# Isabella98Liu/DG-Mesh

Measured on AMD Instinct MI355X. Metric: train-step iters/sec (800x800, ~100k Gaussians), higher is better.
Workload: dtype f32 (f16x3p split products, fp32 accumulate); 1 GPU; D-NeRF jumpingjacks-like cfg2: 800x800, P=100000 Gaussians, deformation MLP on (deform + deform_back, is_blender), 1 frame per rank per step, fixed P (no densification inside the timed region); output heads of both networks scaled x0.01 so that the deformation field is small as after convergence (default init triples every splat's extent); P=100000, W=800, H=800, num_rendered=2808497, visible=95520, mlp_impl=hip, parallelism=dp1 (frame-parallel, flat-bucket all-reduce 27.8 MB)

## Files before the change

dg-mesh_amd/_lib.py:

```python
import ctypes
import os
import subprocess

_HERE = os.path.dirname(os.path.abspath(__file__))
LIB_PATH = os.environ.get("DGM_LIB_PATH") or os.path.join(_HERE, "lib", "libdgmesh_hip.so")
CSRC = os.path.join(_HERE, "csrc")

_c = ctypes
_vp = _c.c_void_p
ALLOC_FN = _c.CFUNCTYPE(_c.c_void_p, _c.c_void_p, _c.c_size_t)


class StateLayout(_c.Structure):
    _fields_ = [(n, _c.c_size_t) for n in (
        "rec", "depth", "radii", "tiles_touched", "offs", "cov3D", "clamped", "block_sums", "hist",
        "tile_count", "tile_offset", "big_list", "counters", "geometry_bytes",
        "inst", "point_list", "slab", "live", "ckpt", "ckpt64", "ulist_full", "binning_bytes",
        "final_T", "n_contrib", "ranges", "nproc", "cfin", "ulist_last", "image_bytes")] + [
        (n, _c.c_int) for n in ("tiles_x", "tiles_y", "n_chunks", "chunk_size")]


class MlpParams(_c.Structure):
    _fields_ = [(n, _c.c_int) for n in ("n_layers", "width", "emb_dim", "t_dim", "skip_layer", "n_out")] + [
        ("W", _vp * 8), ("b", _vp * 8), ("Wh", _vp), ("bh", _vp)]


_f, _i = _c.c_float, _c.c_int
SYMBOLS = {
    "dgm_abi_version": (_i, []),
    "dgm_last_error": (_c.c_char_p, []),
    "dgm_rasterize_forward": (_i, [ALLOC_FN, _vp, ALLOC_FN, _vp, ALLOC_FN, _vp, _i, _i, _i, _vp, _i, _i, _vp, _vp, _vp,
                                   _vp, _vp, _f, _vp, _vp, _vp, _vp, _vp, _f, _f, _i, _vp, _vp, _i, _vp,
                                   _c.POINTER(_i)]),
    "dgm_rasterize_backward": (_i, [_i, _i, _i, _i, _vp, _i, _i, _vp, _vp, _vp, _vp, _f, _vp, _vp, _vp, _vp, _vp, _f, _f,
                                    _vp, _vp, _vp, _vp, _vp, _vp, _vp, _vp, _vp, _vp, _vp, _vp, _vp, _vp, _i, _vp]),
    "dgm_rasterize_forward_split_sh": (_i, [ALLOC_FN, _vp, ALLOC_FN, _vp, ALLOC_FN, _vp, _i, _i, _i, _vp, _i, _i, _vp, _vp, _vp,
                                            _vp, _vp, _vp, _f, _vp, _vp, _vp, _vp, _vp, _f, _f, _i, _vp, _vp, _i, _vp,
                                            _c.POINTER(_i)]),
    "dgm_rasterize_forward_capacity": (_i, [ALLOC_FN, _vp, ALLOC_FN, _vp, ALLOC_FN, _vp, _i, _i, _i, _vp, _i, _i, _vp, _vp, _vp,
                                            _vp, _vp, _vp, _f, _vp, _vp, _vp, _vp, _vp, _f, _f, _i, _vp, _vp, _i, _vp,
                                            _i, _vp]),
    "dgm_rasterize_backward_split_sh": (_i, [_i, _i, _i, _i, _vp, _i, _i, _vp, _vp, _vp, _vp, _vp, _f, _vp, _vp, _vp, _vp,
                                             _vp, _f, _f, _vp, _vp, _vp, _vp, _vp, _vp, _vp, _vp, _vp, _vp, _vp, _vp, _vp,
                                             _vp, _vp, _i, _vp]),
    "dgm_mark_visible": (_i, [_i, _vp, _vp, _vp, _vp, _vp]),
    "dgm_geometry_bytes": (_c.c_size_t, [_i, _i, _i]),
    "dgm_binning_bytes": (_c.c_size_t, [_i]),
    "dgm_image_bytes": (_c.c_size_t, [_i, _i]),
    "dgm_describe_state": (_i, [_i, _i, _i, _i, _c.POINTER(StateLayout)]),
    "dgm_set_profiling": (None, [_i]),
    "dgm_set_profiling_sampling": (None, [_i]),
    "dgm_get_stage_ms": (_i, [_c.POINTER(_f), _i]),
    "dgm_collect_stage_ms": (_i, [_c.POINTER(_f), _c.POINTER(_i), _i]),
    "dgm_stage_name": (_c.c_char_p, [_i]),
    "dgm_knn_scratch_bytes": (_c.c_size_t, [_i]),
    "dgm_knn_mean_dist2": (_i, [_i, _vp, _vp, _vp, _vp]),
    "dgm_image_loss_workspace_bytes": (_c.c_size_t, [_i, _i, _i]),
    "dgm_image_loss_forward": (_i, [_vp, _vp, _i, _i, _i, _f, _vp, _vp, _vp]),
    "dgm_image_loss_backward": (_i, [_vp, _vp, _i, _i, _i, _f, _vp, _vp, _vp, _vp]),
    "dgm_image_metrics_workspace_bytes": (_c.c_size_t, [_i, _i, _i, _i, _i]),
    "dgm_image_metrics": (_i, [_vp, _vp, _i, _i, _i, _i, _f, _i, _vp, _vp, _vp]),
    "dgm_lpips_workspace_bytes": (_c.c_size_t, [_i, _i, _i, _i]),
    "dgm_lpips": (_i, [_i, _c.POINTER(_vp), _c.POINTER(_vp), _c.POINTER(_vp), _vp, _vp, _i, _i, _i, _vp, _vp, _vp]),
    "dgm_gaussian_apply_forward": (_i, [_i, _vp, _vp, _vp, _vp, _vp, _i, _vp, _vp, _vp, _vp, _vp]),
    "dgm_gaussian_apply_backward": (_i, [_i, _vp, _vp, _vp, _vp, _vp, _vp, _vp, _vp, _vp, _vp, _vp, _vp, _i, _vp]),
    "dgm_se3_exp_forward": (_i, [_i, _vp, _i, _vp, _vp]),
    "dgm_se3_exp_backward": (_i, [_i, _vp, _i, _vp, _vp, _i, _vp]),
    "dgm_se3_transform_forward": (_i, [_i, _vp, _vp, _vp, _vp]),
    "dgm_se3_transform_backward": (_i, [_i, _vp, _vp, _vp, _vp, _vp, _vp]),
    "dgm_cycle_loss_workspace_bytes": (_c.c_size_t, [_i]),
    "dgm_cycle_loss_forward": (_i, [_i, _vp, _vp, _i, _vp, _vp, _vp]),
    "dgm_cycle_loss_backward": (_i, [_i, _vp, _vp, _i, _vp, _vp, _vp, _vp]),
    "dgm_adam_step": (_i, [_i, _vp, _vp, _vp, _vp, _vp, _vp, _vp, _f, _f, _f, _vp]),
    "dgm_densify_stats": (_i, [_i, _vp, _vp, _vp, _vp, _vp, _vp]),
    "dgm_densify_scratch_bytes": (_c.c_size_t, [_i]),
    "dgm_densify_totals_offset": (_c.c_size_t, [_i]),
    "dgm_densify_decide": (_i, [_i, _vp, _vp, _vp, _vp, _f, _f, _f, _f, _vp, _vp, _vp]),
# ... 3 lines not shown
    "dgm_dpsr_interp_forward": (_i, [_i, _i, _vp, _vp, _vp, _vp]),
    "dgm_dpsr_interp_backward": (_i, [_i, _i, _vp, _vp, _vp, _vp, _vp, _vp]),
    "dgm_dpsr_spectral": (_i, [_i, _f, _vp, _vp, _i, _vp]),
    "dgm_laplace_scratch_floats": (_c.c_size_t, [_i]),
    "dgm_laplace_forward": (_i, [_i, _i, _vp, _vp, _vp, _vp, _vp]),
    "dgm_laplace_backward": (_i, [_i, _i, _vp, _vp, _vp, _vp, _vp]),
    "dgm_opacity_field_scratch_bytes": (_c.c_size_t, [_i]),
    "dgm_opacity_field": (_i, [_i, _vp, _vp, _vp, _vp, _f, _i, _i, _f, _vp, _vp, _vp, _vp]),
    "dgm_mc_scratch_bytes": (_c.c_size_t, [_i, _i, _i]),
    "dgm_mc_count": (_i, [_i, _i, _i, _vp, _f, _vp, _vp, _vp]),
    "dgm_mc_emit": (_i, [_i, _i, _i, _vp, _vp, _f, _i, _vp, _i, _i, _vp, _vp, _vp]),
    "dgm_mc_backward": (_i, [_i, _i, _i, _vp, _vp, _f, _i, _vp, _i, _vp, _vp, _vp, _vp]),
    "dgm_tri_raster_scratch_bytes": (_c.c_size_t, [_i, _i, _i]),
    "dgm_tri_rasterize_forward": (_i, [_i, _i, _i, _i, _vp, _vp, _vp, _vp, _vp]),
    "dgm_tri_rasterize_backward": (_i, [_i, _i, _i, _i, _vp, _vp, _vp, _vp, _vp, _vp]),
    "dgm_tri_interpolate_forward": (_i, [_i, _i, _i, _i, _i, _vp, _vp, _vp, _vp, _vp]),
    "dgm_tri_interpolate_backward": (_i, [_i, _i, _i, _i, _i, _vp, _vp, _vp, _vp, _vp, _vp, _vp]),
    "dgm_tri_aa_scratch_bytes": (_c.c_size_t, [_i]),
    "dgm_tri_antialias_forward": (_i, [_i, _i, _i, _i, _i, _vp, _vp, _vp, _vp, _vp, _vp, _vp]),
    "dgm_tri_antialias_backward": (_i, [_i, _i, _i, _i, _i, _vp, _vp, _vp, _vp, _vp, _vp, _vp, _vp, _vp]),
    "dgm_anchor_face_geometry": (_i, [_i, _i, _vp, _vp, _vp, _vp, _vp]),
    "dgm_anchor_nn_scratch_bytes": (_c.c_size_t, [_i, _i]),
    "dgm_anchor_nn": (_i, [_i, _i, _vp, _vp, _f, _vp, _vp, _vp, _vp]),
    "dgm_anchor_classify_scratch_bytes": (_c.c_size_t, [_i, _i]),
    "dgm_anchor_classify": (_i, [_i, _i, _vp, _vp, _vp, _vp, _vp, _vp, _vp, _vp, _vp]),
    "dgm_ninit_bbox_scratch_bytes": (_c.c_size_t, []),
    "dgm_ninit_bbox": (_i, [_i, _vp, _vp, _vp, _vp, _vp]),
    "dgm_ninit_face_areas": (_i, [_i, _i, _vp, _vp, _vp, _vp]),
    "dgm_ninit_scan_scratch_bytes": (_c.c_size_t, [_i]),
    "dgm_ninit_area_scan": (_i, [_i, _vp, _vp, _vp, _vp]),
    "dgm_ninit_sample": (_i, [_i, _i, _i, _vp, _vp, _vp, _vp, _vp, _vp, _vp]),
    "dgm_vertex_normals": (_i, [_i, _i, _vp, _vp, _vp, _vp]),
    "dgm_mesh_shade": (_i, [_i, _i, _i, _i, _vp, _vp, _vp, _vp, _vp, _vp, _vp]),
    "dgm_point_splat_scratch_bytes": (_c.c_size_t, [_i, _i]),
    "dgm_point_splat": (_i, [_i, _i, _i, _vp, _vp, _i, _c.POINTER(_f), _vp, _vp, _vp]),
    "dgm_compose_frame": (_i, [_i, _c.POINTER(_vp), _c.POINTER(_i), _i, _i, _i, _vp, _vp]),
    "dgm_emd_tile": (_i, [_i]),
    "dgm_emd_parts": (_i, [_i, _i]),
    "dgm_emd_scratch_floats": (_c.c_size_t, [_i, _i, _i]),
    "dgm_emd_approx": (_i, [_i, _i, _i, _vp, _vp, _vp, _vp, _vp, _vp]),
    "dgm_png_unfilter": (_i, [_i, _i, _i, _i, _vp, _vp, _vp]),
    "dgm_image_ingest": (_i, [_i, _i, _i, _i, _vp, _c.POINTER(_f), _vp, _vp, _vp]),
    "dgm_png_expand": (_i, [_i, _i, _i, _i, _i, _vp, _vp, _vp]),
    "dgm_image_ingest_masked": (_i, [_i, _i, _i, _i, _vp, _i, _vp, _c.POINTER(_f), _i, _vp, _vp, _vp, _vp]),
    "dgm_image_composite_bytes": (_i, [_i, _i, _i, _i, _vp, _c.POINTER(_f), _vp, _vp]),
    "dgm_resample": (_i, [_i, _i, _i, _i, _vp, _i, _i, _vp, _vp, _i, _vp, _vp, _i, _i, _vp, _vp, _vp, _vp, _vp]),
    "dgm_resample_nearest": (_i, [_i, _i, _i, _i, _vp, _i, _i, _vp, _vp, _vp, _vp]),
    "dgm_mlp_set_gemm": (_i, [_i]),
    "dgm_timenet_forward": (_i, [_vp, _i, _vp, _vp, _i, _vp, _vp, _i, _vp, _vp, _vp]),
    "dgm_timenet_backward": (_i, [_vp, _i, _vp, _i, _i, _vp, _vp, _vp, _vp, _vp, _vp]),
    "dgm_mlp_workspace_bytes": (_c.c_size_t, [_i]),
    "dgm_mlp_describe_workspace": (_i, [_i, _c.POINTER(_c.c_size_t), _i]),
    "dgm_mlp_forward": (_i, [_c.POINTER(MlpParams), _i, _vp, _vp, _i, _vp, _vp, _vp]),
    "dgm_mlp_backward": (_i, [_c.POINTER(MlpParams), _i, _vp, _i, _vp, _vp * 8, _vp * 8, _vp, _vp, _vp, _vp]),
    "dgm_mlp_backward_dx": (_i, [_c.POINTER(MlpParams), _i, _vp, _i, _vp, _vp * 8, _vp * 8, _vp, _vp, _vp, _vp, _vp, _vp]),
}

_LIB = None
ABI_VERSION = 5


def build(force=False, verbose=False):
    cmd = ["make", "-C", CSRC, "-j8"] + (["-B"] if force else [])
    out = subprocess.run(cmd, stdout=subprocess.PIPE, stderr=subprocess.STDOUT, text=True)
    if out.returncode != 0:
        raise RuntimeError("building libdgmesh_hip.so failed:\n" + out.stdout[-4000:])
    if verbose:
        print(out.stdout)
    return LIB_PATH


def lib():
    global _LIB
    if _LIB is None:
        if not os.path.exists(LIB_PATH):
            raise RuntimeError(
                f"{LIB_PATH} is missing: build it with `python -c 'import __graft_entry__ as g; g.build()'` "
                "(dg-mesh_amd has no CPU or PyTorch fallback for its kernels)")
        import torch

        handle = ctypes.CDLL(LIB_PATH)
        for name, (res, args) in SYMBOLS.items():
            fn = getattr(handle, name)
            fn.restype = res
            fn.argtypes = args
        if handle.dgm_abi_version() != ABI_VERSION:
            raise RuntimeError(f"libdgmesh_hip.so ABI version {handle.dgm_abi_version()} != {ABI_VERSION} (rebuild: __graft_entry__.build())")
        _LIB = handle
    return _LIB


def stream_ptr():
    import torch
    return ctypes.c_void_p(torch._C._cuda_getCurrentRawStream(torch._C._cuda_getDevice()))


class _NoGuard:
    def __enter__(self):
        return None

    def __exit__(self, *exc):
        return False


_NO_GUARD = _NoGuard()


def device_guard(device):
# ... 27 lines not shown
```

dg-mesh_amd/csrc/c_api.hip:

```cpp
#include <stdarg.h>
#include <stdlib.h>
#include <stdio.h>
#include <string.h>

#include <atomic>
#include <mutex>
#include <string>

#include "dgm_common.hpp"

namespace dgm {
void launch_preprocess_fwd(hipStream_t st, int P, int D, int M, const float* means3D, const float* scales,
                           float scale_modifier, const float* rotations, const float* opacities, const float* shs,
                           const float* shs_rest, const float* cov3D_precomp, const float* colors_precomp,
                           const float* viewmatrix,
                           const float* projmatrix, const float* cam_pos, int W, int H, float tan_fovx, float tan_fovy,
                           int gridx, int gridy, int prefiltered, int* radii_out, float* rec, float* depth,
                           int* radii_int, unsigned* tiles_touched, float* cov3Ds, uint8_t* clamped,
                           unsigned* block_sums);
void launch_mark_visible(hipStream_t st, int P, const float* means3D, const float* viewmatrix, uint8_t* present);
int binning_lds_limit_tiles();
void launch_scan_blocks(hipStream_t st, int n, const unsigned* in, unsigned* out, unsigned* total);
hipError_t launch_count(hipStream_t st, int P, int chunk, int nchunks, int tiles, int gridx,
                        const unsigned* tiles_touched, float* rec, const unsigned* block_sums, unsigned* offs,
                        unsigned* hist, unsigned* counters);
void launch_tile_scan(hipStream_t st, int tiles, int nchunks, unsigned* hist, unsigned* tile_count,
                      unsigned* tile_offset, uint2* ranges, unsigned* big_list, unsigned* big_count, unsigned* arrive,
                      unsigned* total, unsigned capacity, unsigned* tiles_touched, int P);
hipError_t launch_scatter(hipStream_t st, int P, int chunk, int nchunks, int tiles, int gridx, int gridy, size_t R,
                          const unsigned* tiles_touched, const float* rec, const float* depth, const unsigned* hist,
                          const unsigned* tile_offset, uint2* inst);
hipError_t launch_tile_sort(hipStream_t st, int tiles, const uint2* ranges, const uint2* inst, uint2* pairs, size_t R,
                            unsigned* point_list, const unsigned* big_list, const unsigned* big_count, unsigned n_big, unsigned n_mid);
void launch_render_fwd(hipStream_t st, int tiles, const uint2* ranges, const unsigned* point_list, int W, int H,
                       int gridx, const float* rec, const float* bg, float* out_color, float* final_T,
                       unsigned* n_contrib, float4* ckpt, float4* cfin, float4* ckpt64, unsigned* nproc, size_t R, unsigned* uctl,
                       uint4* ulist_full, uint4* ulist_last, uint8_t* live, const unsigned* tile_order);
void launch_render_bwd4(hipStream_t st, int tiles, size_t R, const uint2* ranges, const unsigned* point_list, int W, int H,
                        int gridx, const float* bg, const float* rec, const float4* cfin, const float4* ckpt,
                        const float4* ckpt64, const unsigned* n_contrib, const float* dL_dpix, float* slab,
                        uint8_t* live, const unsigned* uctl, const uint4* ulist_full, const uint4* ulist_last);
void launch_preprocess_bwd(hipStream_t st, int P, int D, int M, int gridx, const float* means3D, const int* radii,
                           const float* shs, const float* shs_rest, const uint8_t* clamped, const float* scales,
                           const float* rotations,
                           float scale_modifier, const float* cov3Ds, const float* viewmatrix, const float* projmatrix,
                           const float* campos, float focal_x, float focal_y, float tan_fovx, float tan_fovy, int W, int H,
                           const float* rec, const unsigned* tiles_touched, const unsigned* offs, const float* slab,
                           const uint8_t* live, float* dL_dmean2D,
                           float* dL_dconic, float* dL_dopacity, float* dL_dcolor, float* dL_dmean3D, float* dL_dcov3D,
                           float* dL_dsh, float* dL_dsh_rest, float* dL_dscale, float* dL_drot);
size_t knn_scratch_bytes(int P);
void launch_knn(hipStream_t st, int P, const float* pts, float* dists, char* scratch);
}

using namespace dgm;

namespace {
thread_local std::string g_err;
}
namespace dgm {
void set_last_error(const char* msg) { g_err = msg ? msg : ""; }
}

namespace {

std::atomic<int> g_profile{0};
float g_stage_ms[DGM_STAGE_COUNT] = {0};
std::mutex g_prof_mu;

struct EventPair {
    hipEvent_t a, b;
};
constexpr int kMaxDeferred = 4096;
EventPair g_deferred[DGM_STAGE_COUNT][kMaxDeferred];
int g_deferred_n[DGM_STAGE_COUNT] = {0};
int g_deferred_created[DGM_STAGE_COUNT] = {0};
int g_sample_every = 1;
int g_calls[DGM_STAGE_COUNT] = {0};
bool g_open[DGM_STAGE_COUNT] = {false};

int fail(const char* fmt, ...) {
    char buf[1024];
    va_list ap;
    va_start(ap, fmt);
    vsnprintf(buf, sizeof(buf), fmt, ap);
    va_end(ap);
    g_err = buf;
    return 1;
}

#define DGM_HIP(call)                                                                                \
    do {                                                                                             \
        hipError_t e_ = (call);                                                                      \
        if (e_ != hipSuccess) return fail("%s failed: %s (%s:%d)", #call, hipGetErrorString(e_), __FILE__, __LINE__); \
    } while (0)

struct StageTimer {
    hipStream_t st;
    int mode;
    hipEvent_t ev[2 * DGM_STAGE_COUNT];
    bool used[DGM_STAGE_COUNT];
    explicit StageTimer(hipStream_t s) : st(s), mode(g_profile) {
        memset(used, 0, sizeof(used));
        if (mode == 1)
            for (auto& e : ev) (void)hipEventCreate(&e);
    }
    void begin(int s) {
        if (mode == 1) {
            (void)hipEventRecord(ev[2 * s], st);
            used[s] = true;
        } else if (mode == 2) {
            std::lock_guard<std::mutex> lk(g_prof_mu);
            if ((g_calls[s]++ % g_sample_every) != 0 || g_deferred_n[s] >= kMaxDeferred) return;
            const int i = g_deferred_n[s];
            if (i >= g_deferred_created[s]) {
                (void)hipEventCreate(&g_deferred[s][i].a);
                (void)hipEventCreate(&g_deferred[s][i].b);
                g_deferred_created[s] = i + 1;
            }
            (void)hipEventRecord(g_deferred[s][i].a, st);
            used[s] = true;
        }
    }
    void end(int s) {
        if (mode == 1) {
            (void)hipEventRecord(ev[2 * s + 1], st);
        } else if (mode == 2 && used[s]) {
            std::lock_guard<std::mutex> lk(g_prof_mu);
            (void)hipEventRecord(g_deferred[s][g_deferred_n[s]].b, st);
            g_deferred_n[s]++;
            used[s] = false;
        }
    }
    void finish() {
        if (mode != 1) return;
        (void)hipStreamSynchronize(st);
        for (int s = 0; s < DGM_STAGE_COUNT; s++)
            if (used[s]) (void)hipEventElapsedTime(&g_stage_ms[s], ev[2 * s], ev[2 * s + 1]);
        for (auto& e : ev) (void)hipEventDestroy(e);
        mode = 0;
    }
    ~StageTimer() { finish(); }
};

}

namespace dgm {
void prof_begin(int s, hipStream_t st) {
    if (g_profile != 2) return;
    std::lock_guard<std::mutex> lk(g_prof_mu);
    g_open[s] = false;
    if ((g_calls[s]++ % g_sample_every) != 0 || g_deferred_n[s] >= kMaxDeferred) return;
    g_open[s] = true;
    const int i = g_deferred_n[s];
    if (i >= g_deferred_created[s]) {
        (void)hipEventCreate(&g_deferred[s][i].a);
        (void)hipEventCreate(&g_deferred[s][i].b);
        g_deferred_created[s] = i + 1;
    }
    (void)hipEventRecord(g_deferred[s][i].a, st);
}
void prof_end(int s, hipStream_t st) {
    if (g_profile != 2) return;
    std::lock_guard<std::mutex> lk(g_prof_mu);
    if (!g_open[s]) return;
    g_open[s] = false;
    if (g_deferred_n[s] >= kMaxDeferred || g_deferred_n[s] >= g_deferred_created[s]) return;
    (void)hipEventRecord(g_deferred[s][g_deferred_n[s]].b, st);
    g_deferred_n[s]++;
}
}

namespace {

int check_launch(const char* what, bool debug, hipStream_t st) {
    hipError_t e = hipGetLastError();
    if (e != hipSuccess) return fail("%s: launch failed: %s", what, hipGetErrorString(e));
    if (debug) {
        e = hipStreamSynchronize(st);
        if (e != hipSuccess) return fail("%s: %s", what, hipGetErrorString(e));
    }
    return 0;
}
#define DGM_CHECK(what)                               \
    do {                                              \
        if (check_launch(what, debug != 0, st)) return 1; \
    } while (0)

}

extern "C" {

int dgm_abi_version(void) { return DGM_ABI_VERSION; }
const char* dgm_last_error(void) { return g_err.c_str(); }

void dgm_set_profiling(int mode) {
    std::lock_guard<std::mutex> lk(g_prof_mu);
    g_profile = mode < 0 ? 0 : (mode > 2 ? 2 : mode);
    if (g_profile == 2)
        for (int s = 0; s < DGM_STAGE_COUNT; s++) g_deferred_n[s] = 0, g_calls[s] = 0, g_open[s] = false;
}
void dgm_set_profiling_sampling(int every) {
    std::lock_guard<std::mutex> lk(g_prof_mu);
    g_sample_every = every < 1 ? 1 : every;
}
int dgm_collect_stage_ms(float* avg_ms, int* counts, int capacity) {
    std::lock_guard<std::mutex> lk(g_prof_mu);
    int n = capacity < DGM_STAGE_COUNT ? capacity : DGM_STAGE_COUNT;
    for (int s = 0; s < n; s++) {
        double tot = 0;
        int ok = 0;
        for (int i = 0; i < g_deferred_n[s]; i++) {
            float ms = 0;
            if (hipEventElapsedTime(&ms, g_deferred[s][i].a, g_deferred[s][i].b) == hipSuccess) {
                tot += ms;
                ok++;
            }
        }
        avg_ms[s] = ok ? (float)(tot / ok) : 0.f;
        if (counts) counts[s] = ok ? g_calls[s] : 0;
        g_deferred_n[s] = 0;
        g_calls[s] = 0;
    }
    return n;
}
int dgm_get_stage_ms(float* ms, int capacity) {
    int n = capacity < DGM_STAGE_COUNT ? capacity : DGM_STAGE_COUNT;
    for (int i = 0; i < n; i++) ms[i] = g_stage_ms[i];
    return n;
}
const char* dgm_stage_name(int s) {
    static const char* names[DGM_STAGE_COUNT] = {"preprocess_fwd", "bin_count",      "bin_scan",      "bin_scatter",
                                                 "tile_sort",      "render_fwd",     "render_bwd",    "preprocess_bwd",
                                                 "mlp_layer_fwd",  "mlp_layer_bwd",  "mlp_layer_dw",  "mlp_bwd_pair"};
    return (s >= 0 && s < DGM_STAGE_COUNT) ? names[s] : "?";
}

size_t dgm_geometry_bytes(int P, int width, int height) {
    dgm_state_layout L;
    compute_layout(P, width, height, 0, &L);
    return L.geometry_bytes;
}
size_t dgm_binning_bytes(int R) {
    dgm_state_layout L;
    compute_layout(0, 16, 16, R, &L);
    return L.binning_bytes;
}
size_t dgm_image_bytes(int width, int height) {
    dgm_state_layout L;
    compute_layout(0, width, height, 0, &L);
    return L.image_bytes;
}
int dgm_describe_state(int P, int width, int height, int R, dgm_state_layout* out) {
    if (!out) return fail("dgm_describe_state: out is NULL");
    compute_layout(P, width, height, R, out);
    return 0;
}

int dgm_rasterize_forward(dgm_alloc_fn geom_alloc, void* geom_ctx, dgm_alloc_fn binning_alloc, void* binning_ctx,
                          dgm_alloc_fn image_alloc, void* image_ctx, int P, int D, int M, const float* background,
                          int width, int height, const float* means3D, const float* shs, const float* colors_precomp,
                          const float* opacities, const float* scales, float scale_modifier, const float* rotations,
                          const float* cov3D_precomp, const float* viewmatrix, const float* projmatrix,
                          const float* cam_pos, float tan_fovx, float tan_fovy, int prefiltered, float* out_color,
                          int* radii, int debug, void* stream, int* num_rendered) {
    return dgm_rasterize_forward_split_sh(geom_alloc, geom_ctx, binning_alloc, binning_ctx, image_alloc, image_ctx, P, D, M,
                                          background, width, height, means3D, shs, nullptr, colors_precomp, opacities, scales,
                                          scale_modifier, rotations, cov3D_precomp, viewmatrix, projmatrix, cam_pos, tan_fovx,
                                          tan_fovy, prefiltered, out_color, radii, debug, stream, num_rendered);
// ... 276 lines not shown
```

dg-mesh_amd/csrc/mlp.hip:

```cpp
#include <stdlib.h>
#include <string.h>

#include "dgm_common.hpp"
#include "mlp_planes.hpp"
#include "mlp_planes5.hpp"

namespace dgm {

static constexpr int MLP_W = 256;
static constexpr int MLP_EMB = 96;
static constexpr int MLP_XE = 63;
static constexpr int GM = 64, GK = 16, GAP = 66;
static constexpr int DW_ROWS = 512;
static constexpr int DW_SLAB = 128;
static constexpr int HD_ROWS = 256;

__global__ void mlp_prep_kernel(int in_features, int Kp, int emb_dim, int is_skip, const float* __restrict__ W,
                                float* __restrict__ Wt, float* __restrict__ Wd) {
    const int idx = blockIdx.x * blockDim.x + threadIdx.x;
    if (idx < Kp * MLP_W) {
        const int k = idx / MLP_W, j = idx % MLP_W;
        int src = -1;
        if (Kp == MLP_W) src = k;
        else if (k < MLP_EMB) src = k < emb_dim ? k : -1;
// ... 207 lines not shown
                                     float* __restrict__ dW, float* __restrict__ db) {
    const int idx = blockIdx.x * blockDim.x + threadIdx.x;
    if (idx < Kp * MLP_W) {
        const int k = idx / MLP_W, j = idx % MLP_W;
        int dst;
        if (Kp == MLP_W) dst = k;
        else if (k < MLP_EMB) dst = k < emb_dim ? k : -1;
        else dst = k - MLP_EMB + emb_dim;
        if (dst >= 0) {
            float sp[16];
#pragma unroll
            for (int u = 0; u < 16; u++) sp[u] = 0.f;
            const float* src = partial + (size_t)k * MLP_W + j;
            const size_t cs = (size_t)Kp * MLP_W;
            int c = 0;
            for (; c + 16 <= chunks; c += 16) {
#pragma unroll
                for (int u = 0; u < 16; u++) sp[u] += src[(size_t)(c + u) * cs];
            }
            for (; c < chunks; c++) sp[0] += src[(size_t)c * cs];
#pragma unroll
            for (int u = 8; u >= 1; u >>= 1)
#pragma unroll
                for (int v = 0; v < u; v++) sp[v] += sp[v + u];
            const float s = sp[0];
            dW[(size_t)j * in_features + dst] = s;
        }
    }
    if (idx < MLP_W && db != nullptr) {
        float sp[8];
#pragma unroll
        for (int u = 0; u < 8; u++) sp[u] = 0.f;
        int c = 0;
        for (; c + 8 <= db_chunks; c += 8) {
#pragma unroll
            for (int u = 0; u < 8; u++) sp[u] += partial_db[(size_t)(c + u) * MLP_W + idx];
        }
        for (; c < db_chunks; c++) sp[0] += partial_db[(size_t)c * MLP_W + idx];
        db[idx] = ((sp[0] + sp[1]) + (sp[2] + sp[3])) + ((sp[4] + sp[5]) + (sp[6] + sp[7]));
    }
}

struct ReduceDwJob {
    int chunks, db_rows, Kp, in_features, nblocks;
    int emb_rows, k_valid;
    int dst_off;
    const float* partial;
    const float* partial_db;
    float* dW;
    float* db;
};
struct ReduceDwBatch {
    int emb_dim, n_jobs;
    ReduceDwJob job[9];
    int h_chunks, h_bchunks, h_nout;
    const float* h_partial_W;
    const float* h_partial_b;
    float* h_dW;
    float* h_db;
};
__device__ __forceinline__ void reduce_heads_body(int bx, int o, int chunks, int bchunks, const float* __restrict__ partial_W,
                                                  const float* __restrict__ partial_b, float* __restrict__ dWh,
                                                  float* __restrict__ dbh);
#ifndef RDW_KT
#define RDW_KT 4
#endif
static constexpr int RDW_JT = 256 / RDW_KT;
static inline int reduce_dw_blocks(int Kp) { return (Kp / RDW_KT) * (MLP_W / RDW_JT); }
__global__ void __launch_bounds__(256)
mlp_reduce_dw_all_kernel(const ReduceDwBatch rb) {
    constexpr int KT = RDW_KT, JT = RDW_JT, JQ = JT / 4, JB = MLP_W / JT;
    __shared__ float4 red[4][64];
    __shared__ float redb[32][8];
    if ((int)blockIdx.y == rb.n_jobs) {
        if ((int)blockIdx.x < 8 * rb.h_nout)
            reduce_heads_body(blockIdx.x & 7, blockIdx.x >> 3, rb.h_chunks, rb.h_bchunks, rb.h_partial_W, rb.h_partial_b, rb.h_dW, rb.h_db);
        return;
    }
    const ReduceDwJob& jb = rb.job[blockIdx.y];
    if ((int)blockIdx.x >= jb.nblocks) return;
    const int chunks = jb.chunks, db_rows = jb.db_rows, Kp = jb.Kp, in_features = jb.in_features, emb_dim = rb.emb_dim;
    const float* __restrict__ partial = jb.partial;
    const float* __restrict__ partial_db = jb.partial_db;
    float* __restrict__ dW = jb.dW;
    float* __restrict__ db = jb.db;
    const int tid = threadIdx.x, pos = tid & 63, grp = tid >> 6;
    const int k0 = ((int)blockIdx.x / JB) * KT, j0 = ((int)blockIdx.x % JB) * JT;
    {
        const int k = k0 + pos / JQ, j = j0 + (pos % JQ) * 4;
        const int per = (chunks + 3) >> 2;
        const int c1 = min(chunks, (grp + 1) * per);
        int c = grp * per;
        const size_t cs = (size_t)Kp * MLP_W;
        const float* src = partial + (size_t)k * MLP_W + j;
        float4 sp[16];
#pragma unroll
        for (int u = 0; u < 16; u++) sp[u] = make_float4(0.f, 0.f, 0.f, 0.f);
        for (; c + 16 <= c1; c += 16) {
            float4 v[16];
#pragma unroll
            for (int u = 0; u < 16; u++) v[u] = *reinterpret_cast<const float4*>(src + (size_t)(c + u) * cs);
#pragma unroll
            for (int u = 0; u < 16; u++) sp[u].x += v[u].x, sp[u].y += v[u].y, sp[u].z += v[u].z, sp[u].w += v[u].w;
        }
        for (; c < c1; c++) {
            const float4 v = *reinterpret_cast<const float4*>(src + (size_t)c * cs);
            sp[0].x += v.x, sp[0].y += v.y, sp[0].z += v.z, sp[0].w += v.w;
        }
#pragma unroll
        for (int u = 8; u >= 1; u >>= 1)
#pragma unroll
            for (int v = 0; v < u; v++)
                sp[v].x += sp[v + u].x, sp[v].y += sp[v + u].y, sp[v].z += sp[v + u].z, sp[v].w += sp[v + u].w;
        red[grp][pos] = sp[0];
    }
    const bool do_db = db != nullptr && blockIdx.x < 32;
    if (do_db) {
        const int col = blockIdx.x * 8 + (tid & 7), g32 = tid >> 3;
        float s = 0.f;
        for (int r = g32; r < db_rows; r += 32) s += partial_db[(size_t)r * MLP_W + col];
        redb[g32][tid & 7] = s;
    }
    __syncthreads();
    {
        const int kk = tid % KT, jj = tid / KT;
        const float* r = reinterpret_cast<const float*>(&red[0][0]) + (kk * JQ + (jj >> 2)) * 4 + (jj & 3);
        const float s = ((r[0] + r[256]) + r[512]) + r[768];
        const int k = k0 + kk;
        int dst;
// ... 207 lines not shown
        for (int i = 0; i < n_pe; i++) a += W1[j * n_pe + i] * pe[i];
        a = fmaxf(a, 0.f);
        h[j] = a;
        save[n_pe + j] = a;
    }
    __syncthreads();
    for (int o0 = 0; o0 < n_out; o0 += 32) {
        const int o = o0 + (tid >> 3), l8 = tid & 7;
        float a = 0.f;
        if (o < n_out) {
#pragma unroll 8
            for (int j = l8; j < hidden; j += 8) a += W2[o * hidden + j] * h[j];
        }
        a += __shfl_xor(a, 1, 64);
        a += __shfl_xor(a, 2, 64);
        a += __shfl_xor(a, 4, 64);
        if (l8 == 0 && o < n_out) out[o] = a + b2[o];
    }
}

__global__ void __launch_bounds__(256)
mlp_timenet_bwd_kernel(const float* __restrict__ d_out, int n_freq, const float* __restrict__ W2, int hidden, int n_out,
                       const float* __restrict__ save, float* __restrict__ dW1, float* __restrict__ db1,
                       float* __restrict__ dW2, float* __restrict__ db2) {
    __shared__ float dO[64];
    const int n_pe = 2 * n_freq + 1;
    const int tid = threadIdx.x;
    if (tid < n_out) {
        dO[tid] = d_out[tid];
        db2[tid] = d_out[tid];
    }
    __syncthreads();
    const float* pe = save;
    const float* h = save + n_pe;
    for (int j = tid; j < hidden; j += 256) {
        const float hj = h[j];
        float dh = 0.f;
        for (int o = 0; o < n_out; o++) {
            dh += dO[o] * W2[o * hidden + j];
            dW2[o * hidden + j] = dO[o] * hj;
        }
        dh = hj > 0.f ? dh : 0.f;
        db1[j] = dh;
        for (int i = 0; i < n_pe; i++) dW1[j * n_pe + i] = dh * pe[i];
    }
}

}

using namespace dgm;

namespace dgm {
void set_last_error(const char* msg);
void prof_begin(int stage, hipStream_t st);
void prof_end(int stage, hipStream_t st);
}
namespace {
int mlp_fail(const char* msg) {
    dgm::set_last_error(msg);
    return 1;
}
struct Ws {
    float *emb, *Y[8], *Wt[8], *Wd[8], *Ga, *Gb, *partial, *partial_db, *partial_h, *partial_hb;
    float *partial_l[8], *partial_db_l[8];
    unsigned* mask[8];
    uint4 *Wt3[8], *Wd3[8];
    float *wsc_f[8], *wsc_d[8], *wsc_e;
    int *Eexp, *Yexp[8], *Dexp, *Gexp[2];
    float4* Cin;
    unsigned char* Dp;
    unsigned* matmax;
    uint4 *Wh4f, *Wh4b;
    float *wsc_hf, *wsc_hb;
    float *bias_s[8];
    float *beff[2], *temb_row;
    size_t bytes;
};
int num_cus() {
    static int cache[DGM_MAX_DEVICES] = {0};
    const int slot = current_device_slot();
    if (cache[slot] == 0) {
        int dev = 0, n = 0;
        if (hipGetDevice(&dev) != hipSuccess || hipDeviceGetAttribute(&n, hipDeviceAttributeMultiprocessorCount, dev) != hipSuccess ||
            n <= 0)
            n = 256;
        cache[slot] = n;
    }
    return cache[slot];
}
int g_gemm_mode = [] {
    const char* e = getenv("DGM_MLP_GEMM");
    if (e == nullptr) return 3;
    if (strcmp(e, "f32") == 0) return 1;
    if (strcmp(e, "f16x3p8") == 0) return 4;
    if (strcmp(e, "f16x3p5") == 0) return 5;
    if (strcmp(e, "f16x3p") != 0) fprintf(stderr, "libdgmesh_hip: unknown DGM_MLP_GEMM=\"%s\" (f16x3p | f16x3p8 | f32): using f16x3p\n", e);
    return 3;
}();
struct WsMode {
    const void* ws;
    int mode;
};
WsMode g_ws_mode[64] = {};
unsigned g_ws_next = 0;
void remember_ws_mode(const void* ws, int mode) {
    for (auto& e : g_ws_mode)
        if (e.ws == ws) {
// ... 115 lines not shown
    }
#define P5_LAUNCH(kernel_, cfg_lds_, grid_, st_, args_)                                                                \
    {                                                                                                                  \
        static bool done_[DGM_MAX_DEVICES] = {false};                                                                  \
        if (p4_lds_attr(kernel_, cfg_lds_, &done_[current_device_slot()]) != hipSuccess)                               \
            return mlp_fail("mlp: cannot raise the LDS limit of a plane-path kernel");                                 \
        hipLaunchKernelGGL(kernel_, dim3(grid_), dim3(256), cfg_lds_, st_, args_);                                     \
    }
typedef Gemm4Cfg<16, 1024, 512, 0, false, 8> CfgFwd;
typedef Gemm4Cfg<16, 1024, 512, 2, false, 8> CfgSkip;
typedef Gemm4Cfg<16, 1024, 512, 1, false, 8> CfgBwd;
typedef Gemm4Cfg<6, 384, 192, 0, true, 8> CfgL0;
typedef Gemm4Cfg<16, 1024, 512, 3, false, 1> CfgHeads;
typedef Gemm4Cfg<1, 128, 64, 1, false, 8> CfgG7;
typedef Gemm4Cfg<4, 256, 128, 0, false, 8, true> CfgL0F;
typedef Gemm4Cfg<16, 1024, 512, 0, false, 8, true> CfgFwdC;
typedef Gemm4Cfg<16, 1024, 512, 1, false, 8, true> CfgBwdC;
typedef Gemm4Cfg<16, 1024, 512, 3, false, 1, true> CfgHeadsC;
typedef Gemm4Cfg<1, 128, 64, 1, false, 8, true> CfgG7C;
typedef Gemm5Cfg<0, 0> Cfg5Fwd;
typedef Gemm5Cfg<0, 1> Cfg5Bwd;
typedef Gemm5Cfg<4, 0> Cfg5Skip;
typedef Gemm5Cfg<0, 2> Cfg5FwdH;
typedef Dw4Cfg<2, 8, 256, 128, 1024, 512> CfgDwE64;
typedef Dw4Cfg<8, 8, 1024, 512, 1024, 512> CfgDw;
typedef Dw4Cfg<3, 8, 384, 192, 1024, 512> CfgDwE;
typedef Dw4Cfg<8, 1, 1024, 512, 128, 64> CfgDwH;
#ifndef P4_PAIR_SHARE_NUM
#define P4_PAIR_SHARE_NUM 128
#define P4_PAIR_SHARE_DEN 256
#endif

int p4_exps_limit() {
    static int v = [] {
        const char* e = getenv("DGM_P4_EXPS_LIMIT");
        const int n = e ? atoi(e) : 512;
        return n < 1 ? 1 : (n > 512 ? 512 : n);
    }();
    return v;
}

int p4_pair_split(int ntiles, int gx) {
    static int env = [] {
        const char* e = getenv("DGM_MLP_PAIR");
        return e ? atoi(e) : -1;
    }();
    if (gx < 64 || ntiles < 4 * gx) return 0;
    int n = env >= 0 ? env : (gx * P4_PAIR_SHARE_NUM) / P4_PAIR_SHARE_DEN;
    if (n >= gx) n = gx - 1;
    return n;
}

int forward_planes(const dgm_mlp_params* p, int N, const float* x, const float* temb, int temb_stride, const Ws& w, float* out,
                   hipStream_t st, const bool fold, const bool all5) {
    const P4Plan pl = p4_plan(N);
    const int nt = pl.ntiles, gx = nt < num_cus() ? nt : num_cus();
    const int sk = p->skip_layer;
    const int EW = fold ? 64 : MLP_EMB;
    static const bool heads_env = [] { const char* e = getenv("DGM_MLP_HEADS_FUSED"); return !(e && atoi(e) == 0); }();
    const bool heads_fused = fold && heads_env && p->n_out <= 16;
    AbsMaxBatch am;
    am.n_jobs = fold ? 0 : 9;
    for (int l = 0; l < 8; l++) am.job[l].W = p->W[l], am.job[l].n = MLP_W * layer_in(p, l);
    am.job[8].W = p->Wh, am.job[8].n = p->n_out * MLP_W;
    if (!fold)
        hipLaunchKernelGGL(mlp_embed4_kernel, dim3(nt + 8 * am.n_jobs), dim3(256), 0, st, N, nt, x, temb, temb_stride, p->t_dim,
                           (unsigned char*)w.emb, w.Eexp, am, w.matmax, EW);
    if (fold) {
        Prep4cBatch pc;
        int nc = 0;
        pc.temb = temb, pc.temb_row = w.temb_row, pc.T = p->t_dim;
        auto addc = [&](int mode, int Kp, int ncols, int in_features, int hoff, int k_valid, int col_valid, const float* Wp, uint4* Bp,
                        float* inv_scale, const float* bias_in, float* bias_out, int fold_time = 0) {
            Prep4cJob& q = pc.job[nc++];
            q.fold = fold_time;
            q.j.mode = mode, q.j.Kp = Kp, q.j.ncols = ncols, q.j.in_features = in_features, q.j.emb_dim = p->emb_dim, q.j.hoff = hoff;
            q.j.k_valid = k_valid, q.j.col_valid = col_valid, q.j.W = Wp, q.j.Bp = Bp, q.j.inv_scale = inv_scale;
            q.bias_in = bias_in, q.bias_out = bias_out;
        };
        for (int l = 0; l < 8; l++) {
            const int Kp = l == 0 ? 64 : (l == sk ? 320 : MLP_W);
            addc(0, Kp, MLP_W, layer_in(p, l), 0, MLP_W, MLP_W, p->W[l], w.Wt3[l], w.wsc_f[l], p->b[l], w.bias_s[l], (l == 0 || l == sk) ? 1 : 0);
            if (l >= 1) addc(1, MLP_W, MLP_W, layer_in(p, l), l == sk ? p->emb_dim : 0, MLP_W, MLP_W, p->W[l], w.Wd3[l], w.wsc_d[l], nullptr, nullptr);
        }
        addc(0, MLP_W, 32, MLP_W, 0, MLP_W, p->n_out, p->Wh, w.Wh4f, w.wsc_hf, nullptr, nullptr);
        addc(1, 16, MLP_W, MLP_W, 0, p->n_out, MLP_W, p->Wh, w.Wh4b, w.wsc_hb, nullptr, nullptr);
        static const bool merged = [] { const char* e = getenv("DGM_MLP_EMBED_MERGED"); return !(e && atoi(e) == 0); }();
        if (merged) {
            const int n_prep = (MLP_W / P4C_COLS) * nc;
            hipLaunchKernelGGL(mlp_embed4c_kernel, dim3(n_prep + nt), dim3(256), 0, st, N, x, (unsigned char*)w.emb, w.Eexp, EW, pc, n_prep);
        } else {
            hipLaunchKernelGGL(mlp_embed4_kernel, dim3(nt), dim3(256), 0, st, N, nt, x, temb, temb_stride, p->t_dim,
                               (unsigned char*)w.emb, w.Eexp, am, w.matmax, EW);
            hipLaunchKernelGGL(mlp_prep4c_kernel, dim3(MLP_W / P4C_COLS, nc), dim3(256), 0, st, pc);
        }
    }
    Prep4Batch pb;
    int nj = 0;
    auto add = [&](int mode, int Kp, int ncols, int in_features, int hoff, int k_valid, int col_valid, const float* Wp, uint4* Bp,
                   float* inv_scale, int mat) {
        Prep4Job& q = pb.job[nj++];
        q.j.mode = mode, q.j.Kp = Kp, q.j.ncols = ncols, q.j.in_features = in_features, q.j.emb_dim = p->emb_dim, q.j.hoff = hoff;
        q.j.k_valid = k_valid, q.j.col_valid = col_valid, q.j.W = Wp, q.j.Bp = Bp, q.j.inv_scale = inv_scale, q.mat = mat;
    };
    for (int l = 0; l < 8; l++) {
        if (fold && l == 0) add(0, 64, MLP_W, layer_in(p, l), 0, MLP_W, MLP_W, p->W[l], w.Wt3[l], w.wsc_f[l], l);
        else if (fold && l == sk) add(0, 320, MLP_W, layer_in(p, l), 0, MLP_W, MLP_W, p->W[l], w.Wt3[l], w.wsc_f[l], l);
        else if (l == sk) {
            add(0, MLP_EMB, MLP_W, layer_in(p, l), 0, MLP_W, MLP_W, p->W[l], w.Wt3[l], w.wsc_e, l);
            add(0, MLP_W, MLP_W, layer_in(p, l), p->emb_dim, MLP_W, MLP_W, p->W[l], w.Wt3[l] + (size_t)MLP_EMB * MLP_W / 4, w.wsc_f[l], l);
        } else
            add(0, layer_kp(p, l), MLP_W, layer_in(p, l), 0, MLP_W, MLP_W, p->W[l], w.Wt3[l], w.wsc_f[l], l);
        if (l >= 1) add(1, MLP_W, MLP_W, layer_in(p, l), l == sk ? p->emb_dim : 0, MLP_W, MLP_W, p->W[l], w.Wd3[l], w.wsc_d[l], l);
    }
    add(0, MLP_W, 32, MLP_W, 0, MLP_W, p->n_out, p->Wh, w.Wh4f, w.wsc_hf, 8);
    add(1, 16, MLP_W, MLP_W, 0, p->n_out, MLP_W, p->Wh, w.Wh4b, w.wsc_hb, 8);
    if (!fold) hipLaunchKernelGGL(mlp_prep4_kernel, dim3(8, nj), dim3(256), 0, st, pb, w.matmax);

    Gemm4Args a;
    memset(&a, 0, sizeof(a));
    a.ntiles = nt, a.M = N, a.exps_limit = p4_exps_limit();
    if (fold) {
        a.A = (const unsigned char*)w.emb, a.Aexp = w.Eexp, a.Bp = w.Wt3[0], a.b_inv = w.wsc_f[0], a.bias = w.bias_s[0];
        a.mask_out = w.mask[0], a.C = (unsigned char*)w.Y[0], a.Cexp = w.Yexp[0];
        P4_LAUNCH((mlp_gemm4_kernel<4, 256, 128, 0, false, 8, true>), CfgL0F::LDS, gx, st, a)
        Gemm5Args b;
        memset(&b, 0, sizeof(b));
        b.ntiles = nt, b.M = N, b.exps_limit = p4_exps_limit();
        for (int l = 1; l < 8; l++) {
            b.A = (const unsigned char*)w.Y[l - 1], b.Aexp = w.Yexp[l - 1], b.Bp = w.Wt3[l], b.b_inv = w.wsc_f[l];
            b.mask_out = w.mask[l], b.C = (unsigned char*)w.Y[l], b.Cexp = w.Yexp[l];
            if (l == sk) {
                b.A2 = (const unsigned char*)w.emb, b.A2exp = w.Eexp, b.bias = w.bias_s[sk];
                P5_LAUNCH((mlp_gemm5_kernel<4, 0>), Cfg5Skip::LDS, gx, st, b)
                b.A2 = nullptr, b.A2exp = nullptr;
            } else if (l == 7 && heads_fused) {
                b.bias = w.bias_s[l];
                b.hBp = w.Wh4f, b.h_inv = w.wsc_hf, b.h_bias = p->bh, b.h_out = out, b.h_nout = p->n_out;
                P5_LAUNCH((mlp_gemm5_kernel<0, 2>), Cfg5FwdH::LDS, gx, st, b)
            } else if (all5) {
                b.bias = w.bias_s[l];
                dgm::prof_begin(DGM_STAGE_MLP_LAYER_FWD, st);
                P5_LAUNCH((mlp_gemm5_kernel<0, 0>), Cfg5Fwd::LDS, gx, st, b)
                dgm::prof_end(DGM_STAGE_MLP_LAYER_FWD, st);
            } else {
                a.A = b.A, a.Aexp = b.Aexp, a.Bp = b.Bp, a.b_inv = b.b_inv, a.bias = w.bias_s[l], a.mask_out = b.mask_out, a.C = b.C, a.Cexp = b.Cexp;
// ... 106 lines not shown
            else P4_LAUNCH((mlp_dw4_kernel<3, 8, 384, 192, 1024, 512>), CfgDwE::LDS, pl.chunks, st, d)
        }
        if (l != 0) {
            d.tiles_per_chunk = paired ? tpc_pair : pl.tiles_per_chunk;
            d.X = (const unsigned char*)w.Y[l - 1], d.Xexp = w.Yexp[l - 1];
            d.partial = part_trunk, d.chunk_stride = stride_trunk;
            d.partial_db = l == sk ? nullptr : w.partial_db_l[l];
        }
        if (paired) {
            dgm::prof_begin(DGM_STAGE_MLP_BWD_PAIR, st);
            {
                static bool done_[DGM_MAX_DEVICES] = {false}, donec_[DGM_MAX_DEVICES] = {false};
                constexpr int LDS_PAIR = CfgBwdC::LDS > CfgDw::LDS ? CfgBwdC::LDS : CfgDw::LDS;
                if ((fold ? p4_lds_attr(mlp_bwd_pair_kernel<true>, LDS_PAIR, &donec_[current_device_slot()])
                          : p4_lds_attr(mlp_bwd_pair_kernel<false>, LDS_PAIR, &done_[current_device_slot()])) != hipSuccess)
                    return mlp_fail("mlp: cannot raise the LDS limit of mlp_bwd_pair_kernel");
                const int grid = n_dw + (gx - n_dw > 0 ? gx - n_dw : 1);
                static const int chunk_env = [] { const char* e = getenv("DGM_MLP_PAIR_CHUNKED"); return e ? atoi(e) : 1; }();
                const int chunked = (chunk_env && grid - n_dw == n_dw && (n_dw % 8) == 0) ? 1 : 0;
                if (fold) hipLaunchKernelGGL(mlp_bwd_pair_kernel<true>, dim3(grid), dim3(512), LDS_PAIR, st, a, d, n_dw, chunked);
                else hipLaunchKernelGGL(mlp_bwd_pair_kernel<false>, dim3(grid), dim3(512), LDS_PAIR, st, a, d, n_dw, chunked);
            }
            dgm::prof_end(DGM_STAGE_MLP_BWD_PAIR, st);
        } else if (l >= 1) {
            dgm::prof_begin(DGM_STAGE_MLP_LAYER_BWD, st);
            if (all5) {
                Gemm5Args b;
                memset(&b, 0, sizeof(b));
                b.ntiles = nt, b.M = N, b.exps_limit = a.exps_limit;
                b.A = a.A, b.Aexp = a.Aexp, b.Bp = a.Bp, b.b_inv = a.b_inv, b.mask_in = a.mask_in, b.C = a.C, b.Cexp = a.Cexp;
                P5_LAUNCH((mlp_gemm5_kernel<0, 1>), Cfg5Bwd::LDS, gx, st, b)
            } else if (fold)
                P4_LAUNCH((mlp_gemm4_kernel<16, 1024, 512, 1, false, 8, true>), CfgBwdC::LDS, gx, st, a)
            else
                P4_LAUNCH((mlp_gemm4_kernel<16, 1024, 512, 1, false, 8>), CfgBwd::LDS, gx, st, a)
            dgm::prof_end(DGM_STAGE_MLP_LAYER_BWD, st);
            dgm::prof_begin(DGM_STAGE_MLP_LAYER_DW, st);
            P4_LAUNCH((mlp_dw4_kernel<8, 8, 1024, 512, 1024, 512>), CfgDw::LDS, chunks_l, st, d)
            dgm::prof_end(DGM_STAGE_MLP_LAYER_DW, st);
        }
        if (paired && l == sk) {
            add_job(n_pending++, pl.chunks, 8 * pl.chunks, EW, layer_in(p, l), 0, part_emb, w.partial_db_l[l], dW[l], db[l]);
            add_job(n_pending++, chunks_l, 0, MLP_W, layer_in(p, l), p->emb_dim, part_trunk, nullptr, dW[l], nullptr);
        } else
            add_job(n_pending++, chunks_l, 8 * chunks_l, Kp, layer_in(p, l), 0, w.partial_l[l], w.partial_db_l[l], dW[l], db[l]);
        if (l >= 1) {
            unsigned char* t = G;
            G = Gn, Gn = t;
            int* te = Ge;
            Ge = Gne, Gne = te;
        }
    }
    rb.n_jobs = n_pending;
    rb.h_chunks = pl.chunks, rb.h_bchunks = nt, rb.h_nout = p->n_out, rb.h_partial_W = w.partial_h, rb.h_partial_b = w.partial_hb;
    rb.h_dW = dWh, rb.h_db = dbh;
    hipLaunchKernelGGL(mlp_reduce_dw_all_kernel, dim3(rb_blocks, rb.n_jobs + 1), dim3(256), 0, st, rb);
    if (fold) {
        FoldGradArgs f;
        f.dW[0] = dW[0], f.db[0] = db[0], f.W[0] = p->W[0], f.in_features[0] = layer_in(p, 0);
        f.dW[1] = dW[sk], f.db[1] = db[sk], f.W[1] = p->W[sk], f.in_features[1] = layer_in(p, sk);
        f.temb = w.temb_row, f.T = p->t_dim, f.dtemb = (dtemb != nullptr && !per_row_t) ? dtemb : nullptr;
        hipLaunchKernelGGL(mlp_fold_grad_kernel, dim3(f.dtemb != nullptr ? 3 : 2, p->t_dim), dim3(256), 0, st, f);
    } else if (dtemb != nullptr && !per_row_t)
        hipLaunchKernelGGL(mlp_dtemb_bcast_kernel, dim3(p->t_dim), dim3(256), 0, st, p->t_dim, db[0], p->W[0], layer_in(p, 0),
                           db[sk], p->W[sk], layer_in(p, sk), dtemb);
    hipError_t e = hipGetLastError();
    if (e != hipSuccess) return mlp_fail(hipGetErrorString(e));
    return 0;
}
}

extern "C" {

int dgm_mlp_set_gemm(int mode) {
    const int prev = g_gemm_mode;
    if (mode == 1 || mode == 3 || mode == 4 || mode == 5) g_gemm_mode = mode;
    return prev;
}

size_t dgm_mlp_workspace_bytes(int N) {
    Ws w = carve(nullptr, N > 0 ? N : 0);
    return w.bytes;
}

#ifdef P4_TIMING
int dgm_p4_timing(unsigned long long* out) {
    return (int)hipMemcpyFromSymbol(out, HIP_SYMBOL(dgm::g_p4_timing), sizeof(unsigned long long) * 256 * 8 * 16);
}
#endif

#ifdef P4_PROBE
namespace {
__global__ void p4_probe_fill_kernel(unsigned* __restrict__ p, size_t n, unsigned seed, int zero) {
    for (size_t i = blockIdx.x * (size_t)blockDim.x + threadIdx.x; i < n; i += (size_t)gridDim.x * blockDim.x) {
        unsigned x = (unsigned)i * 2654435761u + seed;
        x ^= x >> 15, x *= 0x2c1b3c6du, x ^= x >> 12;
        p[i] = zero ? 0u : (x & 0xbfffbfffu);
    }
}
}
int dgm_p4_probe(int N, int kind, int iters, int zero, void* stream) {
    hipStream_t st = (hipStream_t)stream;
    const P4Plan pl = p4_plan(N);
    const int nt = pl.ntiles, gx = nt < num_cus() ? nt : num_cus();
    static unsigned char *A = nullptr, *C = nullptr, *G = nullptr;
    static int* ex = nullptr;
    static uint4* Bp = nullptr;
    static float *binv = nullptr, *bias = nullptr, *partial = nullptr, *pdb = nullptr;
    static unsigned* mask = nullptr;
    static int cap = 0;
    const size_t rows = (size_t)nt * 32;
    if (cap < nt) {
        if (hipMalloc((void**)&A, rows * 1024) != hipSuccess || hipMalloc((void**)&C, rows * 1024) != hipSuccess ||
            hipMalloc((void**)&G, rows * 1024) != hipSuccess || hipMalloc((void**)&ex, (size_t)nt * 4 * 4) != hipSuccess ||
            hipMalloc((void**)&Bp, 16 * 4 * 256 * 16) != hipSuccess || hipMalloc((void**)&binv, 1024) != hipSuccess ||
            hipMalloc((void**)&bias, 1024) != hipSuccess || hipMalloc((void**)&mask, (size_t)nt * 1024) != hipSuccess ||
            hipMalloc((void**)&partial, (size_t)256 * 256 * 256 * 4) != hipSuccess || hipMalloc((void**)&pdb, (size_t)256 * 8 * 256 * 4) != hipSuccess)
            return mlp_fail("p4_probe: hipMalloc failed");
// ... 39 lines not shown
        } else if (kind == 1) {
            P4_LAUNCH((mlp_dw4_kernel<8, 8, 1024, 512, 1024, 512>), CfgDw::LDS, pl.chunks, st, d)
        } else {
            if (n_dw <= 0) return mlp_fail("p4_probe: no pair split at this size");
            static bool done_[DGM_MAX_DEVICES] = {false};
            constexpr int LDS_PAIR = CfgBwd::LDS > CfgDw::LDS ? CfgBwd::LDS : CfgDw::LDS;
            if (p4_lds_attr(mlp_bwd_pair_kernel<false>, LDS_PAIR, &done_[current_device_slot()]) != hipSuccess) return mlp_fail("p4_probe: LDS attribute");
            Dw4Args dp = d;
            dp.tiles_per_chunk = (nt + n_dw - 1) / n_dw;
#ifdef P4_XCD_REDUCE
            {
                static unsigned* xs = nullptr;
                static float* xp = nullptr;
                static int gen = 0;
                if (!xs) {
                    if (hipMalloc((void**)&xs, 8 * 128) != hipSuccess || hipMalloc((void**)&xp, (size_t)8 * 65536 * 4) != hipSuccess) return mlp_fail("p4_probe: hipMalloc");
                    (void)hipMemsetAsync(xs, 0, 8 * 128, st);
                }
                dp.xsync = getenv("DGM_P4_XCD_OFF") ? nullptr : xs, dp.xpartial = xp, dp.xgen = gen++, dp.xchunks = (nt + dp.tiles_per_chunk - 1) / dp.tiles_per_chunk;
            }
#endif
            const int grid = n_dw + (gx - n_dw > 0 ? gx - n_dw : 1);
            const int chunked = (grid - n_dw == n_dw && (n_dw % 8) == 0) ? 1 : 0;
            hipLaunchKernelGGL(mlp_bwd_pair_kernel<false>, dim3(grid), dim3(512), LDS_PAIR, st, a, dp, n_dw, chunked);
        }
    }
    hipError_t e = hipGetLastError();
    if (e != hipSuccess) return mlp_fail(hipGetErrorString(e));
    return 0;
}
#endif

int dgm_mlp_describe_workspace(int N, size_t* offs, int capacity) {
    Ws w = carve(nullptr, N > 0 ? N : 0);
    const char* base = nullptr;
    const void* f[DGM_MLP_WS_FIELDS];
    int n = 0;
    f[n++] = w.emb;
    for (int l = 0; l < 8; l++) f[n++] = w.Y[l];
    for (int l = 0; l < 8; l++) f[n++] = w.mask[l];
    f[n++] = w.Ga, f[n++] = w.Gb;
    f[n++] = w.Eexp;
    for (int l = 0; l < 8; l++) f[n++] = w.Yexp[l];
    f[n++] = w.Dexp, f[n++] = w.Gexp[0], f[n++] = w.Gexp[1];
    f[n++] = w.Cin, f[n++] = w.Dp;
    for (int l = 0; l < 8; l++) f[n++] = w.partial_l[l];
    for (int l = 0; l < 8; l++) f[n++] = w.partial_db_l[l];
    for (int i = 0; i < n && i < capacity; i++) offs[i] = (size_t)((const char*)f[i] - base);
    return n;
}

int dgm_mlp_forward(const dgm_mlp_params* p, int N, const float* x, const float* temb, int temb_stride, char* workspace,
                    float* out, void* stream) {
    if (check_params(p)) return 1;
    if (N <= 0) return 0;
    if (!x || !temb || !workspace || !out) return mlp_fail("mlp_forward: NULL pointer");
    hipStream_t st = (hipStream_t)stream;
    Ws w = carve(workspace, N);
    const int mode = g_gemm_mode;
    const bool fold = (mode == 3 || mode == 5) && temb_stride == 0;
    remember_ws_mode(workspace, mode + (fold ? 16 : 0));
    if (mode >= 3) return forward_planes(p, N, x, temb, temb_stride, w, out, st, fold, fold && mode == 5);
    for (int l = 0; l < 8; l++) {
        const int Kp = layer_kp(p, l);
        const int n = (Kp > MLP_W ? Kp : MLP_W) * MLP_W;
        hipLaunchKernelGGL(mlp_prep_kernel, dim3((n + 255) / 256), dim3(256), 0, st, layer_in(p, l), Kp, p->emb_dim,
                           l == p->skip_layer ? 1 : 0, p->W[l], w.Wt[l], l >= 1 ? w.Wd[l] : nullptr);
    }
    hipLaunchKernelGGL(mlp_embed_kernel, dim3((N + 7) / 8), dim3(256), 0, st, N, x, temb, temb_stride, p->t_dim, w.emb);
    const int grid = (N + GM - 1) / GM;
    for (int l = 0; l < 8; l++) {
        const float *A1, *A2 = nullptr;
        int lda1, K1, lda2 = 0, K2 = 0;
        if (l == 0) {
            A1 = w.emb, lda1 = MLP_EMB, K1 = MLP_EMB;
        } else if (l == p->skip_layer) {
            A1 = w.emb, lda1 = MLP_EMB, K1 = MLP_EMB, A2 = w.Y[l - 1], lda2 = MLP_W, K2 = MLP_W;
        } else {
            A1 = w.Y[l - 1], lda1 = MLP_W, K1 = MLP_W;
        }
        hipLaunchKernelGGL(mlp_gemm_kernel<0>, dim3(grid, MLP_W / GN), dim3(256), 0, st, N, A1, lda1, K1, A2, lda2, K2, w.Wt[l],
                           p->b[l], w.mask[l], w.Y[l]);
    }
    hipLaunchKernelGGL(mlp_rows_small_kernel, dim3((N * 4 + 255) / 256), dim3(256), 0, st, N, p->n_out, w.Y[7], p->Wh, 1,
                       MLP_W, p->bh, out, p->n_out, 0);
    hipError_t e = hipGetLastError();
    if (e != hipSuccess) return mlp_fail(hipGetErrorString(e));
    return 0;
}

int dgm_mlp_backward(const dgm_mlp_params* p, int N, const float* dOut, int temb_stride, char* workspace, float* const* dW,
                     float* const* db, float* dWh, float* dbh, float* dtemb, void* stream) {
    return dgm_mlp_backward_dx(p, N, dOut, temb_stride, workspace, dW, db, dWh, dbh, dtemb, nullptr, nullptr, stream);
}

int dgm_mlp_backward_dx(const dgm_mlp_params* p, int N, const float* dOut, int temb_stride, char* workspace, float* const* dW,
                        float* const* db, float* dWh, float* dbh, float* dtemb, const float* x, float* dX, void* stream) {
    if (check_params(p)) return 1;
    if (N <= 0) return 0;
    if (!dOut || !workspace || !dW || !db || !dWh || !dbh) return mlp_fail("mlp_backward: NULL pointer");
    if ((x == nullptr) != (dX == nullptr)) return mlp_fail("mlp_backward: x and dX come together");
    const int mode = g_gemm_mode;
    if (dX && (mode < 3 || temb_stride != 0))
        return mlp_fail("mlp_backward: the gradient w.r.t. the positions exists in the plane arithmetic only (f16x3p, broadcast time row)");
    {
        const int fm = recall_ws_mode(workspace);
        if (fm >= 0 && (fm & 15) != mode)
            return mlp_fail("mlp_backward: the arithmetic mode changed since the forward pass on this workspace (dgm_mlp_set_gemm)");
        if (fm >= 0 && ((fm & 16) != 0) != ((mode == 3 || mode == 5) && temb_stride == 0))
            return mlp_fail("mlp_backward: temb_stride differs from the forward pass on this workspace");
    }
    hipStream_t st = (hipStream_t)stream;
    Ws w = carve(workspace, N);
    if (mode >= 3) {
        const bool fold = (mode == 3 || mode == 5) && temb_stride == 0;
        return backward_planes(p, N, dOut, temb_stride, w, dW, db, dWh, dbh, dtemb, st, fold, fold && mode == 5, x, dX);
    }
    const int chunks = (N + DW_ROWS - 1) / DW_ROWS;
    const int grid = (N + GM - 1) / GM;
    const int hchunks = (N + HD_ROWS - 1) / HD_ROWS;
    hipLaunchKernelGGL(mlp_heads_bwd_kernel, dim3(hchunks), dim3(256), 0, st, N, p->n_out, dOut, p->Wh, w.Y[7], w.Ga,
                       w.partial_h, w.partial_hb);
    hipLaunchKernelGGL(mlp_reduce_heads_kernel, dim3(8, p->n_out), dim3(256), 0, st, hchunks, p->n_out, w.partial_h,
                       w.partial_hb, dWh, dbh);
    float* G = w.Ga;
    float* Gn = w.Gb;
    const bool per_row_t = temb_stride != 0 && dtemb != nullptr;
    for (int l = 7; l >= 0; l--) {
        const float *X1, *X2 = nullptr;
        int ldx1, K1, ldx2 = 0, K2 = 0;
        if (l == 0) {
            X1 = w.emb, ldx1 = MLP_EMB, K1 = MLP_EMB;
        } else if (l == p->skip_layer) {
            X1 = w.emb, ldx1 = MLP_EMB, K1 = MLP_EMB, X2 = w.Y[l - 1], ldx2 = MLP_W, K2 = MLP_W;
        } else {
            X1 = w.Y[l - 1], ldx1 = MLP_W, K1 = MLP_W;
        }
        if (l >= 1)
            hipLaunchKernelGGL(mlp_gemm_kernel<1>, dim3(grid, MLP_W / GN), dim3(256), 0, st, N, G, MLP_W, MLP_W,
                               (const float*)nullptr, 0, 0, w.Wd[l], (const float*)nullptr, w.mask[l - 1], Gn);
        const int Kp = K1 + K2;
        const int slabs = (Kp + DW_SLAB - 1) / DW_SLAB;
        hipLaunchKernelGGL(mlp_dw_kernel, dim3(slabs, chunks), dim3(512), 0, st, N, X1, ldx1, K1, X2, ldx2, K2, G, w.partial,
                           w.partial_db);
        hipLaunchKernelGGL(mlp_reduce_dw_kernel, dim3((Kp * MLP_W + 255) / 256), dim3(256), 0, st, chunks, chunks, Kp,
                           layer_in(p, l), p->emb_dim, w.partial, w.partial_db, dW[l], db[l]);
        if (per_row_t && (l == p->skip_layer || l == 0))
            for (int c0 = 0; c0 < p->t_dim; c0 += 16)
                hipLaunchKernelGGL(mlp_rows_small_kernel, dim3((N * 4 + 255) / 256), dim3(256), 0, st, N,
                                   p->t_dim - c0 < 16 ? p->t_dim - c0 : 16, G, p->W[l] + MLP_XE + c0, layer_in(p, l), 1,
                                   (const float*)nullptr, dtemb + c0, p->t_dim, l == 0 ? 1 : 0);
        if (l >= 1) {
            float* t = G;
            G = Gn;
            Gn = t;
        }
    }
    if (!per_row_t && dtemb != nullptr)
        hipLaunchKernelGGL(mlp_dtemb_bcast_kernel, dim3(p->t_dim), dim3(256), 0, st, p->t_dim, db[0], p->W[0], layer_in(p, 0),
                           db[p->skip_layer], p->W[p->skip_layer], layer_in(p, p->skip_layer), dtemb);
    hipError_t e = hipGetLastError();
    if (e != hipSuccess) return mlp_fail(hipGetErrorString(e));
    return 0;
}

int dgm_timenet_forward(const float* t, int n_freq, const float* W1, const float* b1, int hidden, const float* W2,
                        const float* b2, int n_out, float* save, float* out, void* stream) {
    if (!t || !W1 || !b1 || !W2 || !b2 || !save || !out) return mlp_fail("timenet_forward: NULL pointer");
    if (n_freq < 0 || 2 * n_freq + 1 > 64 || hidden < 1 || hidden > 1024 || n_out < 1 || n_out > 64)
        return mlp_fail("timenet_forward: unsupported size (2 n_freq + 1 <= 64, hidden <= 1024, n_out <= 64)");
    hipLaunchKernelGGL(mlp_timenet_fwd_kernel, dim3(1), dim3(256), 0, (hipStream_t)stream, t, n_freq, W1, b1, hidden, W2, b2,
                       n_out, save, out);
    hipError_t e = hipGetLastError();
    if (e != hipSuccess) return mlp_fail(hipGetErrorString(e));
    return 0;
}

int dgm_timenet_backward(const float* d_out, int n_freq, const float* W2, int hidden, int n_out, const float* save,
                         float* dW1, float* db1, float* dW2, float* db2, void* stream) {
    if (!d_out || !W2 || !save || !dW1 || !db1 || !dW2 || !db2) return mlp_fail("timenet_backward: NULL pointer");
    if (n_freq < 0 || 2 * n_freq + 1 > 64 || hidden < 1 || hidden > 1024 || n_out < 1 || n_out > 64)
        return mlp_fail("timenet_backward: unsupported size");
    hipLaunchKernelGGL(mlp_timenet_bwd_kernel, dim3(1), dim3(256), 0, (hipStream_t)stream, d_out, n_freq, W2, hidden, n_out,
                       save, dW1, db1, dW2, db2);
    hipError_t e = hipGetLastError();
    if (e != hipSuccess) return mlp_fail(hipGetErrorString(e));
    return 0;
}

}
```

dg-mesh_amd/csrc/mlp_planes.hpp:

```cpp
#pragma once
#include <type_traits>

#include "dgm_common.hpp"

namespace dgm {

typedef _Float16 f16x8 __attribute__((ext_vector_type(8)));
typedef _Float16 f16x2 __attribute__((ext_vector_type(2)));
typedef float f32x2 __attribute__((ext_vector_type(2)));
#ifndef DGM_F32X16_DEFINED
#define DGM_F32X16_DEFINED
typedef float f32x16 __attribute__((ext_vector_type(16)));
#endif

__device__ __forceinline__ f16x8 as_f16x8(const uint4 v) { return __builtin_bit_cast(f16x8, v); }

__device__ __forceinline__ void split2h(float a0, float a1, unsigned& h, unsigned& l) {
    const f16x2 hh = __builtin_convertvector((f32x2){a0, a1}, f16x2);
    const float r0 = a0 - (float)hh.x, r1 = a1 - (float)hh.y;
    const f16x2 ll = __builtin_convertvector((f32x2){r0, r1}, f16x2);
    h = __builtin_bit_cast(unsigned, hh);
    l = __builtin_bit_cast(unsigned, ll);
}

// ... 64 lines not shown
    else if (d >= -24) h = 1u << (d + 24);
    else h = 0u;
    return h | (h << 16);
}

__device__ __forceinline__ void p4_split2(float v0, float v1, int e, unsigned& h, unsigned& l) {
    const float x0 = __builtin_amdgcn_ldexpf(v0, e), x1 = __builtin_amdgcn_ldexpf(v1, e);
    const f16x2 hh = __builtin_convertvector((f32x2){x0, x1}, f16x2);
    float r0, r1;
    asm("v_fma_mix_f32 %0, %1, -1.0, %2 op_sel_hi:[1,0,0]" : "=v"(r0) : "v"(hh), "v"(x0));
    asm("v_fma_mix_f32 %0, %1, -1.0, %2 op_sel:[1,0,0] op_sel_hi:[1,0,0]" : "=v"(r1) : "v"(hh), "v"(x1));
    const f16x2 ll = __builtin_convertvector((f32x2){r0, r1}, f16x2);
    h = __builtin_bit_cast(unsigned, hh);
    l = __builtin_bit_cast(unsigned, ll);
}

__device__ __forceinline__ void p4_glds16(const void* gsrc, unsigned lds_dst) {
    unsigned keep;
    asm volatile("s_mov_b32 %0, m0\n\ts_mov_b32 m0, %2\n\ts_nop 0\n\tglobal_load_lds_dwordx4 %1, off\n\ts_mov_b32 m0, %0"
                 : "=&s"(keep)
                 : "v"(gsrc), "s"(lds_dst)
                 : "memory");
}
#ifdef P4_TIMING
__device__ unsigned long long g_p4_timing[256 * 8 * 16];
#define P4_T(k_)                                                                        \
    {                                                                                   \
        const unsigned long long now_ = __builtin_amdgcn_s_memtime();                   \
        if (P4_TIME_ON) tacc[k_] += now_ - tlast;                                       \
        tlast = now_;                                                                   \
    }
#else
#define P4_T(k_)
#endif
#define P4_LDS_BARRIER() asm volatile("s_waitcnt lgkmcnt(0)\n\ts_barrier" ::: "memory")
#define P4_STEP_BARRIER() asm volatile("s_waitcnt vmcnt(0) lgkmcnt(0)\n\ts_barrier" ::: "memory")

__device__ __forceinline__ unsigned p4_lds_addr(const void* p) {
    return (unsigned)(unsigned long)((__attribute__((address_space(3))) const char*)p);
}

struct AbsMaxJob {
    const float* W;
    int n;
};
static constexpr int P4_MAX_MATS = 12;
struct AbsMaxBatch {
    int n_jobs;
    AbsMaxJob job[P4_MAX_MATS];
};

__device__ __forceinline__ void embed4_tile(const int N, const int tile, const float* __restrict__ x, const float* __restrict__ temb,
                                            const int temb_stride, const int T, unsigned char* __restrict__ Ep, int* __restrict__ Eexp,
                                            const int EW, float (*se)[96 + 1], float* smax);
__global__ void __launch_bounds__(256)
mlp_embed4_kernel(int N, int ntiles, const float* __restrict__ x, const float* __restrict__ temb, int temb_stride, int T,
                  unsigned char* __restrict__ Ep, int* __restrict__ Eexp, const AbsMaxBatch am, unsigned* __restrict__ matmax,
                  const int EW) {
    __shared__ float se[32][96 + 1];
    __shared__ float smax[4];
    const int tid = threadIdx.x, lane = tid & 63, wv = tid >> 6;
    constexpr int AS = 8;
    const int n_am = am.n_jobs * AS;
    if ((int)blockIdx.x < n_am) {
        const int job = (int)blockIdx.x / AS, part = (int)blockIdx.x % AS;
        const AbsMaxJob& jb = am.job[job];
        float m = 0.f;
        const int per = ((jb.n + AS - 1) / AS + 3) & ~3;
        const int i0 = part * per, i1 = min(jb.n, i0 + per);
        if ((((uintptr_t)jb.W) & 15) == 0) {
            const float4* p = reinterpret_cast<const float4*>(jb.W + i0);
            const int n4 = i1 > i0 ? (i1 - i0) >> 2 : 0;
            for (int i = tid; i < n4; i += 256) {
                const float4 v = p[i];
                m = fmaxf(fmaxf(m, fmaxf(fabsf(v.x), fabsf(v.y))), fmaxf(fabsf(v.z), fabsf(v.w)));
            }
            for (int i = i0 + n4 * 4 + tid; i < i1; i += 256) m = fmaxf(m, fabsf(jb.W[i]));
        } else {
            for (int i = i0 + tid; i < i1; i += 256) m = fmaxf(m, fabsf(jb.W[i]));
        }
#pragma unroll
        for (int d = 32; d >= 1; d >>= 1) m = fmaxf(m, __shfl_xor(m, d, 64));
        if (lane == 0) smax[wv] = m;
        __syncthreads();
        if (tid == 0) matmax[job * AS + part] = __float_as_uint(fmaxf(fmaxf(smax[0], smax[1]), fmaxf(smax[2], smax[3])));
        return;
    }
    embed4_tile(N, (int)blockIdx.x - n_am, x, temb, temb_stride, T, Ep, Eexp, EW, se, smax);
}
__device__ __forceinline__ void embed4_tile(const int N, const int tile, const float* __restrict__ x, const float* __restrict__ temb,
                                            const int temb_stride, const int T, unsigned char* __restrict__ Ep, int* __restrict__ Eexp,
                                            const int EW, float (*se)[96 + 1], float* smax) {
    const int tid = threadIdx.x, lane = tid & 63, wv = tid >> 6;
    const int r0 = tile * 32;
    float mx = 0.f;
#pragma unroll
    for (int it = 0; it < 4; it++) {
        if (lane < 60) {
            const int sub = lane / 30, p = lane - 30 * sub, rl = 8 * wv + 2 * it + sub, r = r0 + rl;
            const int q = p / 3, a = p - 3 * q;
            float sn = 0.f, cs = 0.f;
            if (r < N) sincosf(x[3 * r + a] * (float)(1 << q), &sn, &cs);
            se[rl][3 + 6 * q + a] = sn;
            se[rl][6 + 6 * q + a] = cs;
        }
    }
    const int rest = 3 + EW - 63;
    for (int i = tid; i < 32 * rest; i += 256) {
        const int rl = i / rest, j = i - rest * rl, r = r0 + rl;
        float v = 0.f;
        int c;
        if (j < 3) {
            c = j;
            if (r < N) v = x[3 * r + j];
        } else {
            const int t = j - 3;
            c = 63 + t;
            if (EW == 96 && r < N && t < T) v = temb[(size_t)r * temb_stride + t];
        }
        se[rl][c] = v;
        mx = fmaxf(mx, fabsf(v));
    }
#pragma unroll
    for (int d = 32; d >= 1; d >>= 1) mx = fmaxf(mx, __shfl_xor(mx, d, 64));
    if (lane == 0) smax[wv] = mx;
    __syncthreads();
    const float tm = fmaxf(fmaxf(fmaxf(smax[0], smax[1]), fmaxf(smax[2], smax[3])), 1.0f);
    const int e = p4_exp_from_max_bits(__float_as_uint(tm));
    const float sc = p4_pow2(e);
    if (tid == 0) Eexp[tile] = e;
    const int nq = EW >> 2;
    for (int i = tid; i < 32 * nq; i += 256) {
        const int rl = i / nq, c4 = (i - nq * rl) * 4;
        unsigned h0, l0, h1, l1;
        split2h(se[rl][c4] * sc, se[rl][c4 + 1] * sc, h0, l0);
        split2h(se[rl][c4 + 2] * sc, se[rl][c4 + 3] * sc, h1, l1);
        unsigned char* d = Ep + (size_t)(r0 + rl) * (EW * 4) + c4 * 2;
        *reinterpret_cast<uint2*>(d) = make_uint2(h0, h1);
        *reinterpret_cast<uint2*>(d + EW * 2) = make_uint2(l0, l1);
    }
}

struct Prep4Job {
    Prep3Job j;
    int mat;
};
static constexpr int P4_MAX_JOBS = 20;
struct Prep4Batch {
    Prep4Job job[P4_MAX_JOBS];
};
__global__ void __launch_bounds__(256)
mlp_prep4_kernel(const Prep4Batch b, const unsigned* __restrict__ matmax) {
    const Prep4Job& pj = b.job[blockIdx.y];
    const Prep3Job& j = pj.j;
    if ((int)blockIdx.x * 32 >= j.ncols) return;
    const int tid = threadIdx.x, col = blockIdx.x * 32 + (tid & 31), slot = tid >> 5, nkg = j.Kp >> 3;
    float sc, inv;
    unsigned mb = 0u;
#pragma unroll
    for (int i = 0; i < 8; i++) mb = max(mb, matmax[pj.mat * 8 + i]);
    scale_from_max_bits(mb, sc, inv);
    if (blockIdx.x == 0 && tid == 0) j.inv_scale[0] = inv;
#pragma unroll
    for (int it = 0; it < 6; it++) {
        const int kg = slot + 8 * it;
        if (kg < nkg) {
            float e[8];
// ... 38 lines not shown
#pragma unroll
        for (int i = 0; i < 8; i++) {
            e[it][i] = kg < nkg ? prep3_src(j, kg * 8 + i, col) : 0.f;
            m = fmaxf(m, fabsf(e[it][i]));
        }
    }
    smax[slot][cl] = m;
    if (pj.fold && slot < 8) {
        float sacc = 0.f;
        if (col < j.col_valid) {
            const float* wt = j.W + (size_t)col * j.in_features + 63;
            for (int t = slot; t < b.T; t += 8) sacc = fmaf(wt[t], b.temb[t], sacc);
        }
        sfold[slot][cl] = sacc;
    }
    __syncthreads();
    float cm = smax[0][cl];
#pragma unroll
    for (int q = 1; q < P4C_SLOTS; q++) cm = fmaxf(cm, smax[q][cl]);
    float sc, inv;
    scale_from_max_bits(__float_as_uint(cm), sc, inv);
    if (slot == 0) {
        j.inv_scale[col] = inv;
        if (pj.bias_out != nullptr) {
            float bv = (pj.bias_in != nullptr && col < j.col_valid) ? pj.bias_in[col] : 0.f;
            if (pj.fold && col < j.col_valid)
                bv += ((sfold[0][cl] + sfold[1][cl]) + (sfold[2][cl] + sfold[3][cl])) + ((sfold[4][cl] + sfold[5][cl]) + (sfold[6][cl] + sfold[7][cl]));
            pj.bias_out[col] = bv * sc;
        }
    }
    if (bx == 0 && by == 0 && b.temb_row != nullptr && tid < b.T) b.temb_row[tid] = b.temb[tid];
#pragma unroll
    for (int it = 0; it < P4C_ITERS; it++) {
        const int kg = slot + P4C_SLOTS * it;
        if (kg < nkg) {
            uint4 H, L;
            split2h(e[it][0] * sc, e[it][1] * sc, H.x, L.x);
            split2h(e[it][2] * sc, e[it][3] * sc, H.y, L.y);
            split2h(e[it][4] * sc, e[it][5] * sc, H.z, L.z);
            split2h(e[it][6] * sc, e[it][7] * sc, H.w, L.w);
            uint4* dst = j.Bp + ((size_t)(kg >> 1) * 4 + (kg & 1)) * j.ncols + col;
            dst[0] = H;
            dst[2 * j.ncols] = L;
        }
    }
}

__global__ void __launch_bounds__(256)
mlp_prep4c_kernel(const Prep4cBatch b) {
    prep4c_block(b, (int)blockIdx.x, (int)blockIdx.y);
}
__global__ void __launch_bounds__(256)
mlp_embed4c_kernel(const int N, const float* __restrict__ x, unsigned char* __restrict__ Ep, int* __restrict__ Eexp, const int EW,
                   const Prep4cBatch b, const int n_prep) {
    if ((int)blockIdx.x < n_prep) {
        prep4c_block(b, (int)blockIdx.x % (256 / P4C_COLS), (int)blockIdx.x / (256 / P4C_COLS));
        return;
    }
    __shared__ float se[32][96 + 1];
    __shared__ float smax[4];
    embed4_tile(N, (int)blockIdx.x - n_prep, x, nullptr, 0, 0, Ep, Eexp, EW, se, smax);
}

__global__ void __launch_bounds__(256)
mlp_dout4_kernel(int N, int ntiles, int NC, const float* __restrict__ dOut, unsigned char* __restrict__ Dp, int* __restrict__ Dexp,
                 float* __restrict__ partial_b) {
    const int lane = threadIdx.x & 63, wv = threadIdx.x >> 6;
    const int tile = blockIdx.x * 4 + wv;
    if (tile >= ntiles) return;
    const int rl = lane & 31, hf = lane >> 5, r = tile * 32 + rl;
    float v[8];
    float mx = 0.f;
#pragma unroll
    for (int i = 0; i < 8; i++) {
        const int c = 8 * hf + i;
        v[i] = (r < N && c < NC) ? dOut[(size_t)r * NC + c] : 0.f;
        mx = fmaxf(mx, fabsf(v[i]));
    }
#pragma unroll
    for (int d = 32; d >= 1; d >>= 1) mx = fmaxf(mx, __shfl_xor(mx, d, 64));
    const int e = p4_exp_from_max_bits(__float_as_uint(mx));
    const float sc = p4_pow2(e);
    if (lane == 0) Dexp[tile] = e;
    uint4 H, L;
    split2h(v[0] * sc, v[1] * sc, H.x, L.x);
    split2h(v[2] * sc, v[3] * sc, H.y, L.y);
    split2h(v[4] * sc, v[5] * sc, H.z, L.z);
    split2h(v[6] * sc, v[7] * sc, H.w, L.w);
    unsigned char* d = Dp + (size_t)r * 128 + hf * 16;
    const uint4 z = make_uint4(0u, 0u, 0u, 0u);
    *reinterpret_cast<uint4*>(d) = H;
    *reinterpret_cast<uint4*>(d + 32) = z;
    *reinterpret_cast<uint4*>(d + 64) = L;
    *reinterpret_cast<uint4*>(d + 96) = z;
#pragma unroll
    for (int i = 0; i < 8; i++) {
        float s = v[i];
#pragma unroll
        for (int dd = 16; dd >= 1; dd >>= 1) s += __shfl_xor(s, dd, 64);
        if (rl == 0) partial_b[(size_t)tile * 16 + 8 * hf + i] = s;
    }
}

struct Gemm4Args {
    int ntiles, M;
    const unsigned char* A;
    const int* Aexp;
    const uint4* Bp;
    const float* b_inv;
    const float* bias;
    const unsigned* mask_in;
    unsigned* mask_out;
    unsigned char* C;
    int* Cexp;
    const float4* cin;
    const uint4* Bp2;
    const float* b_inv2;
    const float* bias2;
    float4* out2;
    float* out;
    int ldo, n_valid;
    int exps_limit;
};

template <int KS, int ROWB, int PLANEB, int EPI, bool DUAL, int NCW, bool COLSC = false>
struct Gemm4Cfg {
    static constexpr int PITCH = ROWB + 16;
    static constexpr int ABYTES = 32 * PITCH;
    static constexpr int NBUF = 3;
    static constexpr int A_END = (NBUF * ABYTES + 255) & ~255;
    static constexpr int MI_BYTES = EPI == 1 ? NBUF * 1024 : 0;
    static constexpr bool PLANES_OUT = EPI != 3;
    static constexpr int O_BYTES = PLANES_OUT ? 32768 : 0;
    static constexpr int EXPS = 512;
    static constexpr int LDS = A_END + MI_BYTES + O_BYTES + 2 * 1024 + EXPS * 4 + 64 + 1024 + (COLSC ? 1024 : 0);
};

template <int KS, int ROWB, int PLANEB, int EPI, bool DUAL, int NCW, bool COLSC = false>
__device__ __forceinline__ void gemm4_body(const Gemm4Args& a, const int bx, const int G, unsigned char* smem, const int tiles_in = -1) {
    using Cfg = Gemm4Cfg<KS, ROWB, PLANEB, EPI, DUAL, NCW, COLSC>;
    static_assert(!COLSC || (!DUAL && EPI != 2), "column scales: the round-6 kernel forms only");
    constexpr int PITCH = Cfg::PITCH, ABYTES = Cfg::ABYTES;
    constexpr int LPR = ROWB / 16;
    constexpr int RPI = LPR == 64 ? 1 : 64 / (LPR + 1);
    constexpr int NI = (32 + RPI - 1) / RPI;
    constexpr int NCOLS = NCW * 32;
    static_assert(!DUAL || EPI == 0, "the second output rides along with a ReLU layer");
    unsigned char* Abuf = smem;
    unsigned char* Mibuf = smem + Cfg::A_END;
    unsigned char* Obuf = smem + Cfg::A_END + Cfg::MI_BYTES;
    unsigned* mbuf = reinterpret_cast<unsigned*>(Obuf + Cfg::O_BYTES);
    float* tmaxs = reinterpret_cast<float*>(mbuf + 512);
    int* exps = reinterpret_cast<int*>(tmaxs + 16);
    float* biasl = reinterpret_cast<float*>(exps + Cfg::EXPS);
// ... 422 lines not shown

struct Dw4Args {
    int ntiles, tiles_per_chunk;
    const unsigned char* X;
    const int* Xexp;
    const unsigned char* G;
    const int* Gexp;
    float* partial;
    size_t chunk_stride;
    float* partial_db;
#ifdef P4_XCD_REDUCE
    unsigned* xsync;
    float* xpartial;
    int xgen, xchunks;
#endif
};

__device__ __forceinline__ int dw4_pos(int col) { return (col & ~7) | ((col ^ (col >> 3)) & 7); }
__device__ __forceinline__ unsigned dw4_dword(const uint4& v, int i) { return i == 0 ? v.x : (i == 1 ? v.y : (i == 2 ? v.z : v.w)); }
__device__ __forceinline__ float dw4_dot_ones(unsigned d, float acc) {
    const f16x2 one = {(_Float16)1.0f, (_Float16)1.0f};
    return __builtin_amdgcn_fdot2(__builtin_bit_cast(f16x2, d), one, acc, false);
}
__device__ __forceinline__ unsigned dw4_pk_mul(unsigned d, unsigned f2) {
    return __builtin_bit_cast(unsigned, __builtin_bit_cast(f16x2, d) * __builtin_bit_cast(f16x2, f2));
}

template <int MT, int NT, int XROWB, int XPLANEB, int GROWB, int GPLANEB>
struct Dw4Cfg {
    static constexpr int XK = MT * 32, GK = NT * 32;
    static constexpr int XU = 8 * XK, GU = 8 * GK;
    static constexpr int LDS = 2 * (XU + GU) * 16;
};

template <int MT, int NT, int XROWB, int XPLANEB, int GROWB, int GPLANEB>
__device__ __forceinline__ void dw4_body(const Dw4Args& a, const int chunk, unsigned char* smem) {
    using Cfg = Dw4Cfg<MT, NT, XROWB, XPLANEB, GROWB, GPLANEB>;
    constexpr int XK = Cfg::XK, GK = Cfg::GK, XU = Cfg::XU, GU = Cfg::GU;
    constexpr int XCG = XK / 8, GCG = GK / 8;
    constexpr int XB = XCG * 8, GB = GCG * 8;
    constexpr int MTW = NT == 8 ? MT : 1;
    static_assert(NT == 8 || (NT == 1 && MT == 8), "wave decomposition");
    static_assert(XB <= 256 && GB <= 256, "stager layout");
    uint4* const dw4_lds = reinterpret_cast<uint4*>(smem);
    uint4* Xs = dw4_lds;
    uint4* Gs = dw4_lds + 2 * XU;
    const int tid = threadIdx.x, lane = tid & 63, wv = __builtin_amdgcn_readfirstlane(tid >> 6);
    const int g = lane >> 5, li = lane & 31;
    const int t0 = chunk * a.tiles_per_chunk, t1 = min(a.ntiles, t0 + a.tiles_per_chunk);
    const int nst = t1 - t0;
    if (nst <= 0) return;

    int eref = 0x7fffffff;
    for (int t = t0; t < t1; t++) eref = min(eref, a.Xexp[t] + a.Gexp[t]);
    eref = __builtin_amdgcn_readfirstlane(eref);

    const bool isX = tid < XB, isG = tid >= 256 && tid < 256 + GB;
    const int st = isG ? tid - 256 : tid;
    const int ncg = isG ? GCG : XCG;
#ifndef DW4_ROWMAJOR_STAGERS
#define DW4_ROWMAJOR_STAGERS 1
#endif
    const int cg = st % ncg;
    const int pl = DW4_ROWMAJOR_STAGERS ? (st / ncg) & 1 : st / (ncg * 4);
    const int rg = DW4_ROWMAJOR_STAGERS ? st / (ncg * 2) : (st / ncg) & 3;
    const unsigned char* src = isG ? a.G + (size_t)pl * GPLANEB + cg * 16 : a.X + (size_t)pl * XPLANEB + cg * 16;
    const int srow = isG ? GROWB : XROWB;
    uint4* sdst = (isG ? Gs : Xs) + (pl * 4 + rg) * (isG ? GK : XK) + cg * 8;
    const int sbuf = isG ? GU : XU;
    const int swz = cg & 7;
    uint4 R[8];
    float cs[8];
#pragma unroll
    for (int i = 0; i < 8; i++) cs[i] = 0.f;

#define DW4_LOAD(t_)                                                                                                   \
    if (isX || isG) {                                                                                                  \
        const unsigned char* p_ = src + ((size_t)(t_) * 32 + rg * 8) * srow;                                           \
        _Pragma("unroll") for (int i_ = 0; i_ < 8; i_++) R[i_] = *reinterpret_cast<const uint4*>(p_ + (size_t)i_ * srow); \
    }
#define DW4_STORE(t_, buf_)                                                                                            \
    if (isX || isG) {                                                                                                  \
        const int et_ = a.Xexp[t_] + a.Gexp[t_];                                                                       \
        const unsigned f2_ = p4_pow2_h2(eref - et_);                                                                   \
        const bool scale_ = isX && et_ != eref;                                                                        \
        float tsum_[8];                                                                                                \
        _Pragma("unroll") for (int c_ = 0; c_ < 8; c_++) {                                                             \
            const unsigned sel_ = (c_ & 1) ? 0x07060302u : 0x05040100u;                                                \
            uint4 o_;                                                                                                  \
            o_.x = __builtin_amdgcn_perm(dw4_dword(R[1], c_ >> 1), dw4_dword(R[0], c_ >> 1), sel_);                    \
            o_.y = __builtin_amdgcn_perm(dw4_dword(R[3], c_ >> 1), dw4_dword(R[2], c_ >> 1), sel_);                    \
            o_.z = __builtin_amdgcn_perm(dw4_dword(R[5], c_ >> 1), dw4_dword(R[4], c_ >> 1), sel_);                    \
            o_.w = __builtin_amdgcn_perm(dw4_dword(R[7], c_ >> 1), dw4_dword(R[6], c_ >> 1), sel_);                    \
            if (isG && a.partial_db != nullptr) {                                                                      \
                float s_ = dw4_dot_ones(o_.x, 0.f);                                                                    \
                s_ = dw4_dot_ones(o_.y, s_), s_ = dw4_dot_ones(o_.z, s_), s_ = dw4_dot_ones(o_.w, s_);                 \
                tsum_[c_] = s_;                                                                                        \
            }                                                                                                          \
            if (scale_) o_.x = dw4_pk_mul(o_.x, f2_), o_.y = dw4_pk_mul(o_.y, f2_), o_.z = dw4_pk_mul(o_.z, f2_), o_.w = dw4_pk_mul(o_.w, f2_); \
            sdst[(buf_) * sbuf + (c_ ^ swz)] = o_;                                                                     \
        }                                                                                                              \
        if (isG && a.partial_db != nullptr) {                                                                          \
            const float ig_ = p4_pow2(-a.Gexp[t_]);                                                                    \
            _Pragma("unroll") for (int c_ = 0; c_ < 8; c_++) cs[c_] += tsum_[c_] * ig_;                                \
        }                                                                                                              \
    }

// ... 84 lines not shown
                __builtin_amdgcn_fence(__ATOMIC_ACQUIRE, "agent");
            }
            __syncthreads();
            const int rows_per = (256 + members - 1) / members, r0 = member * rows_per, r1 = min(256, r0 + rows_per);
            for (int i = r0 * 64 + tid; i < r1 * 64; i += 512) {
                float4 sacc = make_float4(0.f, 0.f, 0.f, 0.f);
                for (int m = 0; m < members; m++) {
                    const float4 v = *reinterpret_cast<const float4*>(a.partial + (size_t)(grp + 8 * m) * a.chunk_stride + (size_t)i * 4);
                    sacc.x += v.x, sacc.y += v.y, sacc.z += v.z, sacc.w += v.w;
                }
                *reinterpret_cast<float4*>(a.xpartial + ((size_t)grp * 65536 + (size_t)i * 4)) = sacc;
            }
        }
#endif
    } else {
        if (li < 16) {
#pragma unroll
            for (int r = 0; r < 16; r++) {
                const int c = wv * 32 + (r & 3) + 8 * (r >> 2) + 4 * g;
                a.partial[((size_t)chunk * 16 + li) * 256 + c] = ldexpf(acc[0][r], -eref);
            }
        }
    }
    if (isG && a.partial_db != nullptr) {
        float* d = a.partial_db + ((size_t)chunk * 8 + pl * 4 + rg) * GK + cg * 8;
        *reinterpret_cast<float4*>(d) = make_float4(cs[0], cs[1], cs[2], cs[3]);
        *reinterpret_cast<float4*>(d + 4) = make_float4(cs[4], cs[5], cs[6], cs[7]);
    }
}

template <int MT, int NT, int XROWB, int XPLANEB, int GROWB, int GPLANEB>
__global__ void __launch_bounds__(512)
mlp_dw4_kernel(const Dw4Args a) {
    extern __shared__ __attribute__((aligned(16))) unsigned char p4_smem[];
    dw4_body<MT, NT, XROWB, XPLANEB, GROWB, GPLANEB>(a, (int)blockIdx.x, p4_smem);
}

template <bool COLSC>
__global__ void __launch_bounds__(512)
mlp_bwd_pair_kernel(const Gemm4Args ga, const Dw4Args da, const int n_dw, const int chunked) {
    extern __shared__ __attribute__((aligned(16))) unsigned char p4_smem[];
    if ((int)blockIdx.x < n_dw) {
        dw4_body<8, 8, 1024, 512, 1024, 512>(da, (int)blockIdx.x, p4_smem);
    } else if (chunked) {
        const int w = (int)blockIdx.x - n_dw;
        const int first = w * da.tiles_per_chunk;
        const int cnt = min(da.tiles_per_chunk, ga.ntiles - first);
        gemm4_body<16, 1024, 512, 1, false, 8, COLSC>(ga, first, 1, p4_smem, cnt > 0 ? cnt : 0);
    } else {
        gemm4_body<16, 1024, 512, 1, false, 8, COLSC>(ga, (int)blockIdx.x - n_dw, (int)gridDim.x - n_dw, p4_smem);
    }
}

__global__ void __launch_bounds__(256)
mlp_dx4_kernel(int N, const unsigned char* __restrict__ G, const int* __restrict__ Gexp, const float* __restrict__ W, int in_features,
               int col0, int ncol, float* __restrict__ scratch, int finish, const float* __restrict__ x, float* __restrict__ dX,
               int ldo) {
    __shared__ float sG[32][32 + 1];
    __shared__ float sW[32][64 + 1];
    __shared__ float sE[32][64 + 1];
    const int tile = blockIdx.x, r0 = tile * 32, tid = threadIdx.x;
    const int ty = tid >> 4, tx = tid & 15;
    const float scale = __builtin_ldexpf(1.0f, -Gexp[tile]);
    float acc[2][4] = {{0.f, 0.f, 0.f, 0.f}, {0.f, 0.f, 0.f, 0.f}};
    for (int k0 = 0; k0 < 256; k0 += 32) {
        {
            const int r = tid >> 3, kk = (tid & 7) * 4;
            const unsigned char* row = G + (size_t)(r0 + r) * 1024;
            const uint2 h = *reinterpret_cast<const uint2*>(row + (k0 + kk) * 2);
            const uint2 l = *reinterpret_cast<const uint2*>(row + 512 + (k0 + kk) * 2);
            const f16x2 h0 = __builtin_bit_cast(f16x2, h.x), h1 = __builtin_bit_cast(f16x2, h.y);
            const f16x2 l0 = __builtin_bit_cast(f16x2, l.x), l1 = __builtin_bit_cast(f16x2, l.y);
            sG[r][kk + 0] = (float)h0[0] + (float)l0[0];
            sG[r][kk + 1] = (float)h0[1] + (float)l0[1];
            sG[r][kk + 2] = (float)h1[0] + (float)l1[0];
            sG[r][kk + 3] = (float)h1[1] + (float)l1[1];
        }
        for (int i = tid; i < 32 * 64; i += 256) {
            const int kk = i >> 6, c = i & 63;
            sW[kk][c] = c < ncol ? W[(size_t)(k0 + kk) * in_features + col0 + c] : 0.f;
        }
        __syncthreads();
#pragma unroll 8
        for (int kk = 0; kk < 32; kk++) {
            const float g0 = sG[2 * ty][kk], g1 = sG[2 * ty + 1][kk];
#pragma unroll
            for (int c = 0; c < 4; c++) {
                const float wv = sW[kk][4 * tx + c];
                acc[0][c] = fmaf(g0, wv, acc[0][c]);
                acc[1][c] = fmaf(g1, wv, acc[1][c]);
            }
        }
        __syncthreads();
    }
#pragma unroll
    for (int e = 0; e < 2; e++) {
        const int r = r0 + 2 * ty + e;
        float4 v = make_float4(acc[e][0] * scale, acc[e][1] * scale, acc[e][2] * scale, acc[e][3] * scale);
        float4* sp = reinterpret_cast<float4*>(scratch + (size_t)r * 64 + 4 * tx);
        if (finish) {
            const float4 p = *sp;
            v.x += p.x, v.y += p.y, v.z += p.z, v.w += p.w;
            sE[2 * ty + e][4 * tx + 0] = v.x, sE[2 * ty + e][4 * tx + 1] = v.y, sE[2 * ty + e][4 * tx + 2] = v.z, sE[2 * ty + e][4 * tx + 3] = v.w;
        } else {
            *sp = v;
        }
// ... 30 lines not shown
```

dg-mesh_amd/csrc/mlp_planes5.hpp:

```cpp
#pragma once
#include "mlp_planes.hpp"

#ifndef P5_ABL
#define P5_ABL 0
#endif
#ifndef P5_W_AGPR
#define P5_W_AGPR 12
#endif
#ifndef P5_BQ_AHEAD
#define P5_BQ_AHEAD 1
#endif
#ifndef P5_W_AGPR_SKIP
#define P5_W_AGPR_SKIP 14
#endif

namespace dgm {

struct Gemm5Args {
    int ntiles, M;
    const unsigned char* A;
    const int* Aexp;
    const unsigned char* A2;
    const int* A2exp;
    const uint4* Bp;
// ... 365 lines not shown
            }
            if (j + 1 < my_tiles) {
                const int abn = ab == 2 ? 0 : ab + 1;
                const unsigned char* ps1 = Abuf + abn * ABYTES + li * P1 + g * 16;
                const unsigned char* ps2 = Abuf + abn * ABYTES + A1BYTES + li * P2 + g * 16;
                G5_FRAG(0)
            }
            if (EPI == 0 && P5_BQ_AHEAD) bq = *reinterpret_cast<const float4*>(biasl + (2 * wv) * 32 + 8 * 3 + 4 * g);
        }
        if (HM.value && j + 1 < my_tiles) asm volatile("s_waitcnt lgkmcnt(%0)\n\ts_barrier" ::"n"((EPI == 0 && P5_BQ_AHEAD ? 1 : 0) + 2) : "memory");
        else if (HM.value && EPI == 0 && P5_BQ_AHEAD) asm volatile("s_waitcnt lgkmcnt(1)\n\ts_barrier" ::: "memory");
        else P4_LDS_BARRIER();
    };
    {
        const unsigned char* ps1 = Abuf + li * P1 + g * 16;
        const unsigned char* ps2 = Abuf + A1BYTES + li * P2 + g * 16;
        G5_FRAG(0)
    }
    typedef std::integral_constant<bool, true> T_;
    typedef std::integral_constant<bool, false> F_;
    step(T_{}, F_{}, F_{}, 0, 0);
    if (my_tiles > 1) step(T_{}, T_{}, F_{}, 1, 1);
    int ab = 2;
    for (int j = 2; j < my_tiles; j++) {
        step(T_{}, T_{}, T_{}, j, ab);
        ab = ab == 2 ? 0 : ab + 1;
    }
    if (my_tiles >= 2) step(F_{}, T_{}, T_{}, my_tiles, my_tiles % 3);
    else step(F_{}, T_{}, F_{}, my_tiles, my_tiles % 3);
    step(F_{}, F_{}, T_{}, my_tiles + 1, (my_tiles + 1) % 3);
#undef G5_COPY1
#undef G5_COPY_MASK
#undef G5_FRAG
#undef G5_MFMA
}

template <int KS2, int EPI>
__global__ void __launch_bounds__(256) __attribute__((amdgpu_waves_per_eu(1, 1)))
mlp_gemm5_kernel(const Gemm5Args a) {
    extern __shared__ __attribute__((aligned(16))) unsigned char p4_smem[];
    gemm5_body<KS2, EPI>(a, (int)blockIdx.x, (int)gridDim.x, p4_smem);
}


struct FoldGradArgs {
    float* dW[2];
    const float* db[2];
    const float* W[2];
    int in_features[2];
    const float* temb;
    float* dtemb;
    int T;
};
__global__ void __launch_bounds__(256)
mlp_fold_grad_kernel(const FoldGradArgs f) {
    __shared__ float red[4];
    const int k = blockIdx.x, t = blockIdx.y, j = threadIdx.x;
    if (k < 2) {
        f.dW[k][(size_t)j * f.in_features[k] + 63 + t] = f.db[k][j] * f.temb[t];
        return;
    }
    float v = f.db[0][j] * f.W[0][(size_t)j * f.in_features[0] + 63 + t] + f.db[1][j] * f.W[1][(size_t)j * f.in_features[1] + 63 + t];
#pragma unroll
    for (int d = 32; d >= 1; d >>= 1) v += __shfl_xor(v, d, 64);
    if ((j & 63) == 0) red[j >> 6] = v;
    __syncthreads();
    if (j == 0) f.dtemb[t] = (red[0] + red[1]) + (red[2] + red[3]);
}

}
```

dg-mesh_amd/deform.py:

```python
import math
import os

import numpy as np
import torch
import torch.nn as nn
import torch.nn.functional as F


def positional_encoding(v, n_freqs):
    out = [v]
    freqs = 2.0 ** torch.linspace(0.0, n_freqs - 1, steps=n_freqs)
    for f in freqs:
        out.append(torch.sin(v * f))
        out.append(torch.cos(v * f))
    return torch.cat(out, -1)


def skew(w):
    zeros = torch.zeros(w.shape[0], device=w.device)
    return torch.stack([zeros, -w[:, 2], w[:, 1], w[:, 2], zeros, -w[:, 0], -w[:, 1], w[:, 0], zeros], -1).reshape(-1, 3, 3)


def exp_se3(S, theta):
    w, v = torch.split(S, 3, dim=-1)
# ... 177 lines not shown
class _ModelWrapper:
    net_attr = "deform"

    def __init__(self, net, lr_scale, model_name, final_lr_scale=1.0):
        setattr(self, self.net_attr, net)
        if getattr(net, "trunk_impl", None) == "hip":
            from . import mlp_hip
            mlp_hip.pack_heads(net.head_modules())
        self.optimizer = None
        self.spatial_lr_scale = lr_scale
        self.final_lr_scale = final_lr_scale
        self.model_name = model_name

    @property
    def net(self):
        return getattr(self, self.net_attr)

    def step(self, xyz, time_emb):
        return self.net(xyz, time_emb)

    def step_raw(self, xyz, time_emb):
        net = self.net
        if isinstance(net, DeformNetwork) and not net.is_6dof:
            return net.heads_out(xyz, time_emb)
        return None

    def train_setting(self, training_args):
        lr0 = training_args.position_lr_init * self.spatial_lr_scale
        self.optimizer = torch.optim.Adam([{"params": list(self.net.parameters()), "lr": lr0, "name": self.model_name}],
                                          lr=0.0, eps=1e-15)
        self.scheduler = get_expon_lr_func(lr_init=lr0, lr_final=training_args.position_lr_final * self.final_lr_scale,
                                           lr_delay_mult=training_args.position_lr_delay_mult,
                                           max_steps=training_args.deform_lr_max_steps)

    def update_learning_rate(self, iteration):
        for group in self.optimizer.param_groups:
            if group["name"] == self.model_name:
                lr = self.scheduler(iteration)
                group["lr"] = lr
                return lr

    def save_weights(self, model_path, iteration):
        out = os.path.join(model_path, f"{self.model_name}/iteration_{iteration}")
        os.makedirs(out, exist_ok=True)
        torch.save(self.net.state_dict(), os.path.join(out, f"{self.model_name}.pth"))

    def load_weights(self, model_path, iteration=-1):
        root = os.path.join(model_path, self.model_name)
        if iteration == -1:
            iteration = max(int(f.split("_")[-1]) for f in os.listdir(root))
        self.net.load_state_dict(torch.load(os.path.join(root, f"iteration_{iteration}/{self.model_name}.pth")))


class DeformModel(_ModelWrapper):
    def __init__(self, is_blender=False, is_6dof=False, device="cuda", trunk_impl=None):
        super().__init__(DeformNetwork(is_blender=is_blender, is_6dof=is_6dof, trunk_impl=trunk_impl).to(device), 5, "deform")


class DeformModelNormal(_ModelWrapper):
    def __init__(self, is_blender=False, is_6dof=False, model_name="deform", device="cuda", trunk_impl=None):
        super().__init__(DeformNetworkNormal(is_blender=is_blender, is_6dof=is_6dof, trunk_impl=trunk_impl).to(device), 5,
                         model_name)


class DeformModelNormalSep(_ModelWrapper):
    def __init__(self, is_blender=False, is_6dof=False, model_name="deform_normal", device="cuda", trunk_impl=None):
        super().__init__(DeformNetworkNormalSep(is_blender=is_blender, is_6dof=is_6dof, trunk_impl=trunk_impl).to(device),
                         10.0, model_name, final_lr_scale=10.0)


class AppearanceModel(_ModelWrapper):
    net_attr = "appearance_net"

    def __init__(self, is_blender=False, is_6dof=False, device="cuda", trunk_impl=None):
        super().__init__(AppearanceNetwork(is_blender=is_blender, trunk_impl=trunk_impl).to(device), 1.0, "appearance")

    def train_setting(self, training_args):
        lr0 = training_args.apperance_lr_init
        self.optimizer = torch.optim.Adam([{"params": list(self.net.parameters()), "lr": lr0, "name": "appearance"}],
                                          lr=0.0, eps=1e-15)
        self.scheduler = get_expon_lr_func(lr_init=lr0, lr_final=training_args.apperance_lr_final,
                                           lr_delay_mult=training_args.apperance_lr_delay_mult,
                                           max_steps=training_args.apperance_lr_max_steps)
```

dg-mesh_amd/mlp_hip.py:

```python
import ctypes

import torch

from . import _lib


def _params(net, W, b, Wh, bh, t_dim):
    p = _lib.MlpParams()
    p.n_layers, p.width, p.emb_dim, p.t_dim, p.skip_layer, p.n_out = 8, 256, 63 + t_dim, t_dim, 5, Wh.shape[0]
    for l in range(8):
        p.W[l] = W[l].data_ptr()
        p.b[l] = b[l].data_ptr()
    p.Wh, p.bh = Wh.data_ptr(), bh.data_ptr()
    return p


def _adjacent(ts):
    at = ts[0].data_ptr()
    for t in ts:
        if t.dtype != torch.float32 or not t.is_contiguous() or t.data_ptr() != at:
            return False
        at += 4 * t.numel()
    return True

# ... 26 lines not shown
class _MLPFunction(torch.autograd.Function):

    @staticmethod
    def forward(ctx, x, t_emb, bcast, n_heads, *tensors):
        L = _lib.lib()
        hw, hb, wb = tensors[:n_heads], tensors[n_heads:2 * n_heads], tensors[2 * n_heads:]
        n_out = sum(w.shape[0] for w in hw)
        Wh, bh = _stacked(hw, (n_out, hw[0].shape[1])), _stacked(hb, (n_out,))
        W, b = [w.contiguous() for w in wb[:8]], [v.contiguous() for v in wb[8:]]
        x, t_emb = x.contiguous(), t_emb.contiguous()
        N, T = x.shape[0], t_emb.shape[1]
        ws = torch.empty(L.dgm_mlp_workspace_bytes(N), dtype=torch.uint8, device=x.device)
        out = torch.empty((N, Wh.shape[0]), dtype=torch.float32, device=x.device)
        p = _params(None, W, b, Wh, bh, T)
        st = _lib.stream_ptr()
        with _lib.device_guard(x.device):
            _lib.check(L.dgm_mlp_forward(ctypes.byref(p), N, ctypes.c_void_p(x.data_ptr()), ctypes.c_void_p(t_emb.data_ptr()),
                                         0 if bcast else T, ctypes.c_void_p(ws.data_ptr()), ctypes.c_void_p(out.data_ptr()), st))
        ctx.save_for_backward(ws, Wh, bh, x, *W, *b)
        ctx.meta = (N, T, bool(bcast), t_emb.requires_grad, [w.shape[0] for w in hw])
        return out

    @staticmethod
    def backward(ctx, dOut):
        L = _lib.lib()
        ws, Wh, bh, x, *wb = ctx.saved_tensors
        W, b = wb[:8], wb[8:]
        N, T, bcast, need_t, head_rows = ctx.meta
        dOut = dOut.contiguous()
        dev = dOut.device
        dW = [torch.empty_like(w) for w in W]
        db = [torch.empty_like(v) for v in b]
        dWh, dbh = torch.empty_like(Wh), torch.empty_like(bh)
        dtemb = torch.empty((1, T) if bcast else (N, T), dtype=torch.float32, device=dev)
        p = _params(None, W, b, Wh, bh, T)
        arr = ctypes.c_void_p * 8
        dWp = arr(*[t.data_ptr() for t in dW])
        dbp = arr(*[t.data_ptr() for t in db])
        st = _lib.stream_ptr()
        dX = None
        with _lib.device_guard(dev):
            if ctx.needs_input_grad[0]:
                dX = torch.empty((N, 3), dtype=torch.float32, device=dev)
                _lib.check(L.dgm_mlp_backward_dx(ctypes.byref(p), N, ctypes.c_void_p(dOut.data_ptr()), 0 if bcast else T,
                                                 ctypes.c_void_p(ws.data_ptr()), dWp, dbp, ctypes.c_void_p(dWh.data_ptr()),
                                                 ctypes.c_void_p(dbh.data_ptr()), ctypes.c_void_p(dtemb.data_ptr()),
                                                 ctypes.c_void_p(x.data_ptr()), ctypes.c_void_p(dX.data_ptr()), st))
            else:
                _lib.check(L.dgm_mlp_backward(ctypes.byref(p), N, ctypes.c_void_p(dOut.data_ptr()), 0 if bcast else T,
                                              ctypes.c_void_p(ws.data_ptr()), dWp, dbp, ctypes.c_void_p(dWh.data_ptr()),
                                              ctypes.c_void_p(dbh.data_ptr()), ctypes.c_void_p(dtemb.data_ptr()), st))
        dWs, dbs = torch.split(dWh, head_rows, 0), torch.split(dbh, head_rows, 0)
        return (dX, dtemb if need_t else None, None, None, *dWs, *dbs, *dW, *db)


class _TimeNetFunction(torch.autograd.Function):

    @staticmethod
    def forward(ctx, t, n_freq, W1, b1, W2, b2):
        L = _lib.lib()
        W1, b1, W2, b2 = W1.contiguous(), b1.contiguous(), W2.contiguous(), b2.contiguous()
        t = t.reshape(-1)[:1].contiguous().float()
        hidden, n_out = W1.shape[0], W2.shape[0]
        if W1.shape[1] != 2 * n_freq + 1 or W2.shape[1] != hidden:
            raise RuntimeError("timenet: weight shapes do not match PE(t) / hidden width")
        save = torch.empty(2 * n_freq + 1 + hidden, dtype=torch.float32, device=t.device)
        out = torch.empty((1, n_out), dtype=torch.float32, device=t.device)
        st = _lib.stream_ptr()
        vp = lambda x: ctypes.c_void_p(x.data_ptr())
        with _lib.device_guard(t.device):
            _lib.check(L.dgm_timenet_forward(vp(t), n_freq, vp(W1), vp(b1), hidden, vp(W2), vp(b2), n_out, vp(save), vp(out), st))
        ctx.save_for_backward(save, W1, W2)
        ctx.n_freq = n_freq
        return out

    @staticmethod
    def backward(ctx, d_out):
        L = _lib.lib()
        save, W1, W2 = ctx.saved_tensors
        d_out = d_out.contiguous()
        hidden, n_out = W1.shape[0], W2.shape[0]
        dW1, db1 = torch.empty_like(W1), torch.empty(hidden, dtype=torch.float32, device=W1.device)
        dW2, db2 = torch.empty_like(W2), torch.empty(n_out, dtype=torch.float32, device=W1.device)
        st = _lib.stream_ptr()
        vp = lambda x: ctypes.c_void_p(x.data_ptr())
        with _lib.device_guard(W1.device):
            _lib.check(L.dgm_timenet_backward(vp(d_out), ctx.n_freq, vp(W2), hidden, n_out, vp(save), vp(dW1), vp(db1), vp(dW2),
                                              vp(db2), st))
        return None, None, dW1, db1, dW2, db2


def time_row(net, t_row):
    lin1, lin2 = net.timenet[0], net.timenet[2]
    return _TimeNetFunction.apply(t_row, net.t_multires, lin1.weight, lin1.bias, lin2.weight, lin2.bias)


def check_supported(net, heads, t_emb):
    T = t_emb.shape[1]
    key = (T, tuple(m.weight.shape[0] for m in heads))
    if net.__dict__.get("_dgm_supported") == key:
        return
    in0 = 63 + T
    ok = (getattr(net, "D", None) == 8 and getattr(net, "W", None) == 256 and getattr(net, "multires", None) == 10
          and list(getattr(net, "skips", [])) == [4] and len(net.linear) == 8 and in0 <= 96)
    if ok:
        for l, lin in enumerate(net.linear):
            want = (256, in0) if l == 0 else ((256, 256 + in0) if l == 5 else (256, 256))
            ok = ok and tuple(lin.weight.shape) == want and lin.bias is not None and tuple(lin.bias.shape) == (256,)
        for m in heads:
            ok = ok and m.weight.shape[1] == 256 and m.bias is not None
        ok = ok and 1 <= sum(m.weight.shape[0] for m in heads) <= 16
    if not ok:
        raise RuntimeError("trunk_impl='hip' supports the reference trunk only (D=8, W=256, multires=10, skips=[4], at most "
                           "16 head outputs); build the network with trunk_impl='torch' for other shapes")
    net.__dict__["_dgm_supported"] = key


def network_forward(net, heads, x, t_emb, bcast):
    if not x.is_cuda:
        raise RuntimeError("trunk_impl='hip' needs CUDA/HIP tensors (dg-mesh_amd has no CPU path for its kernels)")
    if x.requires_grad and not bcast:
        raise RuntimeError("trunk_impl='hip' differentiates w.r.t. the positions only with a broadcast time row (the plane "
                           "arithmetic); use trunk_impl='torch' for per-row time inputs")
    if x.requires_grad and _lib.lib().dgm_mlp_set_gemm(-1) not in (3, 4, 5):
        raise RuntimeError("trunk_impl='hip' differentiates w.r.t. the positions only in the default f16x3p arithmetic "
                           "(DGM_MLP_GEMM / dgm_mlp_set_gemm select another one): use trunk_impl='torch' for this network")
    check_supported(net, heads, t_emb)
    W = [l.weight for l in net.linear]
    b = [l.bias for l in net.linear]
    return _MLPFunction.apply(x, t_emb, bcast, len(heads), *[m.weight for m in heads], *[m.bias for m in heads], *W, *b)
```

dg-mesh_amd/trainer.py:

```python
import os
import random

import torch
import torch.distributed as dist

from . import rasterizer as _RZ
from . import scene as S


class FlatGradBucket:

    def __init__(self, params, attach=True):
        self.params = [p for p in params if p.requires_grad]
        total = sum(p.numel() for p in self.params)
        ref = self.params[0]
        self.flat = torch.zeros(total, dtype=ref.dtype, device=ref.device)
        self.views = []
        off = 0
        for p in self.params:
            n = p.numel()
            self.views.append(self.flat[off:off + n].view_as(p))
            if attach:
                p.grad = self.views[-1]
            off += n
# ... 79 lines not shown
        self.init = {"density_thres": density_thres, "center": center, "scale": scale}
        d = torch.randn(n_verts, 3, generator=gen)
        d = d / d.norm(dim=1, keepdim=True)
        self.probes = (0.5 + 0.25 * d * (1 + 0.1 * torch.randn(n_verts, 1, generator=gen))).clamp(0.02, 0.98).to(dev)
        self.verts = None
        self.phi_target = torch.zeros(n_verts, device=dev)
        self.color_target = torch.rand(n_verts, 3, generator=gen).to(dev)

    def bind(self, g):
        with torch.no_grad():
            if self.init["density_thres"] is not None:
                g.density_thres_param.fill_(float(self.init["density_thres"]))
            if self.init["center"] is not None:
                g.gaussian_center = torch.tensor(self.init["center"], dtype=torch.float32, device=g.gaussian_center.device)
            if self.init["scale"] is not None:
                g.gaussian_scale = torch.tensor([float(self.init["scale"])], dtype=torch.float32, device=g.gaussian_scale.device)
        self.verts = ((self.probes * 2.0 - 1.0) * g.gaussian_scale + g.gaussian_center).contiguous()

    def networks(self):
        return [self.deform_normal, self.deform_back_normal, self.appearance]

    def psr(self, g, deform, deform_normal, freeze_pos=False):
        pts = g.get_xyz.detach() + deform.detach() if freeze_pos and deform is not None else (
            g.get_xyz + deform if deform is not None else g.get_xyz)
        pts = ((pts - g.gaussian_center) / g.gaussian_scale) / 2.0 + 0.5
        pts = torch.clamp(pts, 1e-6, 1 - 1e-6)
        normals = g.get_normal + deform_normal if deform_normal is not None else g.get_normal
        psr = self.dpsr(pts.unsqueeze(0), normals.unsqueeze(0))
        sign = torch.where(psr[0, 0, 0, 0].detach() < 0, -1.0, 1.0)
        return (psr * sign - g.density_thres_param)[0]

    def surface(self, g, psr):
        verts, faces = self.diffmc(psr, deform=None, isovalue=0.0)
        verts = verts * 2.0 - 1.0
        return verts * g.gaussian_scale + g.gaussian_center, faces

    @torch.no_grad()
    def extract_mesh(self, g, deform=None, deform_normal=None, t=None):
        if self.dpsr is None:
            raise RuntimeError("MeshPhase.extract_mesh needs the DPSR module")
        xyz = g.get_xyz
        tt = None if t is None else torch.as_tensor(t, dtype=torch.float32, device=xyz.device).reshape(1, 1).expand(xyz.shape[0], -1)
        d_xyz = deform.step(xyz.detach(), tt)[0] if deform is not None else None
        d_normal = deform_normal.step(xyz.detach(), tt) if deform_normal is not None else None
        if isinstance(d_normal, (tuple, list)):
            d_normal = d_normal[0]
        return self.surface(g, self.psr(g, d_xyz, d_normal))


class Trainer:
    def __init__(self, gaussians, deform, deform_back, cameras, opt=None, pipe=None, background=None,
                 is_blender=True, is_6dof=False, rank=0, world=1, seed=0, render_fn=None, fused_adam=None,
                 process_group=None, fused_loss=True, fused_glue=None, track_stats=True, densify=False,
                 cameras_extent=1.0, prune_threshold=0.005, white_background=True, overlap=False, mesh=None):
        self.g, self.deform, self.deform_back = gaussians, deform, deform_back
        self.mesh = mesh
        self.cameras = cameras
        self.opt = opt or S.OptimizationParams()
        self.pipe = pipe or S.PipelineParams()
        self.bg = background
        self.is_blender, self.is_6dof = is_blender, is_6dof
        self.rank, self.world, self.seed = rank, world, seed
        self.render_fn = render_fn or S.render
        self.group = process_group
        self.fused_loss = fused_loss
        self.track_stats = track_stats
        self.densify = densify
        self.overlap = overlap
        self.cameras_extent, self.prune_threshold, self.white_background = cameras_extent, prune_threshold, white_background
        self.step_count = 0
        self.fused_glue = bool(fused_glue) if fused_glue is not None else (
            gaussians.get_xyz.is_cuda and render_fn is None and not is_6dof)
        dev = gaussians.get_xyz.device
        fused = (dev.type == "cuda") if fused_adam is None else fused_adam
        if mesh is not None:
            mesh.bind(gaussians)
        gaussians.training_setup(self.opt)
        deform.train_setting(self.opt)
        deform_back.train_setting(self.opt)
        self.optimizers = [gaussians.optimizer, deform.optimizer, deform_back.optimizer]
        if mesh is not None:
            for m in mesh.networks():
                m.train_setting(self.opt)
                self.optimizers.append(m.optimizer)
        self.multi_adam = None
        if fused:
            from .optim import MultiAdam
            self.multi_adam = MultiAdam(self.optimizers)
        self.pack = self.multi_adam is not None
        self._bind_parameters()
        self.densify_generator = None
        if dev.type == "cuda":
            self.densify_generator = torch.Generator(device=dev)
            self.densify_generator.manual_seed(1234567 + seed)
        self.anchor_generator = None
        self._anchor_plan = None
        self.last_anchor_info = None
        if dev.type == "cuda":
            self.anchor_generator = torch.Generator(device=dev)
            self.anchor_generator.manual_seed(7654321 + seed)
        self.normal_init_generator = None
        if dev.type == "cuda":
            self.normal_init_generator = torch.Generator(device=dev)
            self.normal_init_generator.manual_seed(2468013 + seed)
        self.time_interval = 1.0 / max(len(cameras), 1)
        from .deform import get_linear_noise_func
        self.smooth_term = get_linear_noise_func(lr_init=0.1, lr_final=1e-15, lr_delay_mult=0.01, max_steps=20000)

# ... 105 lines not shown
            dist.all_reduce(self.g.xyz_gradient_accum, op=dist.ReduceOp.SUM, group=self.group)
            dist.all_reduce(self.g.denom, op=dist.ReduceOp.SUM, group=self.group)
            dist.all_reduce(self.g.max_radii2D, op=dist.ReduceOp.MAX, group=self.group)

    def state_hash(self):
        dev = self.g.get_xyz.device
        words = []
        for p in self.params:
            st = None
            for o in self.optimizers:
                if p in o.state:
                    st = o.state[p]
                    break
            for t in (p.detach(), st.get("exp_avg") if st else None, st.get("exp_avg_sq") if st else None):
                if t is None or t.numel() == 0:
                    words.append(torch.zeros((), dtype=torch.int64, device=dev))
                    continue
                bits = t.contiguous().view(torch.int32).reshape(-1).to(torch.int64)
                w = (torch.arange(bits.numel(), device=dev, dtype=torch.int64) * 2654435761 + 0x1E3779B97F4A7C15) | 1
                words.append((bits * w).sum())
        return torch.stack(words)

    def replicas_identical(self):
        h = self.state_hash()
        if self.world == 1:
            return True
        parts = [torch.empty_like(h) for _ in range(self.world)]
        dist.all_gather(parts, h, group=self.group)
        return all(bool(torch.equal(parts[0], q)) for q in parts[1:])

    def bucket_bytes(self):
        if self._early is not None:
            return [self._early[k].nbytes() for k in ("g", "m")]
        return [self.bucket.nbytes()] if self.bucket is not None else [self.grad_bytes()]

    def grad_bytes(self):
        return sum(p.numel() for p in self.params) * 4

    def time_input(self, cam, N, iteration):
        t = cam.fid.reshape(1, 1)
        if not self.is_blender:
            t = t + torch.randn(1, 1, device=t.device) * self.time_interval * self.smooth_term(iteration)
        return t.expand(N, -1)

    def loss_terms(self, cam, iteration):
        g, opt = self.g, self.opt
        delta = None
        if iteration < opt.warm_up:
            d_xyz, d_rotation, d_scaling = 0.0, 0.0, 0.0
        else:
            N = g.get_xyz.shape[0]
            time_input = self.time_input(cam, N, iteration)
            t_back = self.time_input(cam, N, iteration)
            if self.fused_glue:
                delta = self.deform.step_raw(g.get_xyz.detach(), time_input)
            if delta is None:
                d_xyz, d_rotation, d_scaling = self.deform.step(g.get_xyz.detach(), time_input)[:3]
        losses = {}
        if delta is not None:
            from .glue import cycle_loss
            lean = {"lean": True} if self.render_fn is S.render else {}
            if self.world > 1 and self._early is not None:
                means = (g.get_xyz.detach() + delta.detach()[:, :3]).contiguous()
                back = self.deform_back.step_raw(means, t_back)
                losses["cycle_loss"] = cycle_loss(delta, back)
                pkg = self.render_fn(cam, g, self.pipe, self.bg, None, None, None, self.is_6dof, delta=delta, **lean)
            else:
                pkg = self.render_fn(cam, g, self.pipe, self.bg, None, None, None, self.is_6dof, delta=delta, **lean)
                back = self.deform_back.step_raw(pkg["means3D"].detach(), t_back)
                losses["cycle_loss"] = cycle_loss(delta, back)
        else:
            pkg = self.render_fn(cam, g, self.pipe, self.bg, d_xyz, d_rotation, d_scaling, self.is_6dof)
            if iteration >= opt.warm_up:
                deformed_xyz = g.get_xyz + d_xyz
                back = self.deform_back.step(deformed_xyz.detach(), t_back)
                cycle = (S.l1_loss(-back[0], d_xyz) + S.l1_loss(-back[1], d_rotation) + S.l1_loss(-back[2], d_scaling)) / 3.0
                losses["cycle_loss"] = cycle
        if self.normal_init_due(iteration):
            if delta is not None:
                self.normal_init_step(delta[:, :3], delta[:, 3:7], delta[:, 7:10])
            else:
                self.normal_init_step(d_xyz, d_rotation, d_scaling)
        if self.mesh is not None and iteration >= opt.dpsr_iter:
            self.mesh_terms(cam, iteration, losses, pkg, delta if delta is not None else None,
                            None if delta is not None else (d_xyz if iteration >= opt.warm_up else None), time_input, t_back)
        image = pkg["render"]
        gt = cam.original_image
        if image.is_cuda and self.fused_loss:
            from .loss import image_loss
            losses["img_loss"] = image_loss(image, gt, opt.lambda_dssim)
        else:
            Ll1 = S.l1_loss(image, gt)
            losses["img_loss"] = (1.0 - opt.lambda_dssim) * Ll1 + opt.lambda_dssim * (1.0 - S.ssim(image, gt))
        return losses, pkg

    def mesh_terms(self, cam, iteration, losses, pkg, delta, d_xyz, t_fwd, t_back):
        g, opt, ms = self.g, self.opt, self.mesh
        N = g.get_xyz.shape[0]
        xyz_d = g.get_xyz.detach()
        normal_nets = iteration >= opt.dpsr_iter + normal_deform_delay(opt)
        d_normal = ms.deform_normal.step(xyz_d, t_fwd) if normal_nets else None
        if normal_nets:
            d_normal_back = ms.deform_back_normal.step(xyz_d, t_back)
            l_n = S.l1_loss(-d_normal_back, d_normal)
            if "cycle_loss" in losses:
                losses["cycle_loss"] = losses["cycle_loss"] * 0.75 + l_n * 0.25
        if ms.dpsr is None:
            if normal_nets:
                losses["normal_reg"] = (g.get_normal + d_normal).abs().mean() * 1e-3
            return
        dx = delta[:, :3] if delta is not None else d_xyz
        freeze_pos = iteration < opt.dpsr_iter + opt.normal_warm_up
        psr = ms.psr(g, dx, d_normal, freeze_pos=freeze_pos)
        if ms.mesh_source == "diffmc":
            self.diffmc_terms(cam, iteration, losses, psr)
# ... 126 lines not shown
```

include/dgmesh_hip.h:

```cpp
#ifndef DGMESH_HIP_H
#define DGMESH_HIP_H

#include <stddef.h>
#include <stdint.h>

#ifdef __cplusplus
extern "C" {
#endif

#define DGM_ABI_VERSION 5

typedef char* (*dgm_alloc_fn)(void* ctx, size_t bytes);

int dgm_abi_version(void);
const char* dgm_last_error(void);


int dgm_rasterize_forward(dgm_alloc_fn geom_alloc, void* geom_ctx, dgm_alloc_fn binning_alloc, void* binning_ctx,
                          dgm_alloc_fn image_alloc, void* image_ctx, int P, int D, int M, const float* background,
                          int width, int height, const float* means3D, const float* shs, const float* colors_precomp,
                          const float* opacities, const float* scales, float scale_modifier, const float* rotations,
                          const float* cov3D_precomp, const float* viewmatrix, const float* projmatrix,
                          const float* cam_pos, float tan_fovx, float tan_fovy, int prefiltered, float* out_color,
                          int* radii, int debug, void* stream, int* num_rendered);
// ... 74 lines not shown
} dgm_state_layout;

int dgm_describe_state(int P, int width, int height, int R, dgm_state_layout* out);

enum {
    DGM_STAGE_PREPROCESS = 0,
    DGM_STAGE_BIN_COUNT,
    DGM_STAGE_BIN_SCAN,
    DGM_STAGE_BIN_SCATTER,
    DGM_STAGE_TILE_SORT,
    DGM_STAGE_RENDER_FWD,
    DGM_STAGE_RENDER_BWD,
    DGM_STAGE_PREPROCESS_BWD,
    DGM_STAGE_MLP_LAYER_FWD,
    DGM_STAGE_MLP_LAYER_BWD,
    DGM_STAGE_MLP_LAYER_DW,
    DGM_STAGE_MLP_BWD_PAIR,
    DGM_STAGE_COUNT
};
void dgm_set_profiling(int mode);
void dgm_set_profiling_sampling(int every);
int dgm_get_stage_ms(float* ms, int capacity);
int dgm_collect_stage_ms(float* avg_ms, int* counts, int capacity);
const char* dgm_stage_name(int stage);


size_t dgm_knn_scratch_bytes(int P);
int dgm_knn_mean_dist2(int P, const float* points, float* mean_dists, char* scratch, void* stream);


typedef struct {
    int n_layers;
    int width;
    int emb_dim;
    int t_dim;
    int skip_layer;
    int n_out;
    const float* W[8];
    const float* b[8];
    const float* Wh;
    const float* bh;
} dgm_mlp_params;

int dgm_mlp_set_gemm(int mode);

size_t dgm_mlp_workspace_bytes(int N);

#define DGM_MLP_WS_FIELDS 49
int dgm_mlp_describe_workspace(int N, size_t* offs, int capacity);

int dgm_mlp_forward(const dgm_mlp_params* p, int N, const float* x, const float* temb, int temb_stride,
                    char* workspace, float* out, void* stream);

int dgm_mlp_backward(const dgm_mlp_params* p, int N, const float* dOut, int temb_stride, char* workspace,
                     float* const* dW, float* const* db, float* dWh, float* dbh, float* dtemb, void* stream);
int dgm_mlp_backward_dx(const dgm_mlp_params* p, int N, const float* dOut, int temb_stride, char* workspace,
                        float* const* dW, float* const* db, float* dWh, float* dbh, float* dtemb, const float* x, float* dX,
                        void* stream);

int dgm_timenet_forward(const float* t, int n_freq, const float* W1, const float* b1, int hidden, const float* W2,
                        const float* b2, int n_out, float* save, float* out, void* stream);
int dgm_timenet_backward(const float* d_out, int n_freq, const float* W2, int hidden, int n_out, const float* save,
                         float* dW1, float* db1, float* dW2, float* db2, void* stream);


size_t dgm_image_loss_workspace_bytes(int channels, int H, int W);
int dgm_image_loss_forward(const float* image, const float* gt, int channels, int H, int W, float lambda_dssim,
                           char* workspace, float* out, void* stream);
int dgm_image_loss_backward(const float* image, const float* gt, int channels, int H, int W, float lambda_dssim,
                            const char* workspace, const float* grad_out, float* d_image, void* stream);


size_t dgm_image_metrics_workspace_bytes(int B, int C, int H, int W, int levels);
int dgm_image_metrics(const float* images, const float* gt, int B, int C, int H, int W, float data_range, int levels, char* workspace,
                      double* out, void* stream);

size_t dgm_lpips_workspace_bytes(int net, int B, int H, int W);
int dgm_lpips(int net, const float* const* conv_w, const float* const* conv_b, const float* const* lin, const float* images,
              const float* gt, int B, int H, int W, char* workspace, double* out, void* stream);


int dgm_gaussian_apply_forward(int P, const float* xyz, const float* scaling, const float* rotation, const float* opacity,
                               const float* delta, int ld, float* means3D, float* scales, float* rotations,
                               float* opacities, void* stream);
int dgm_gaussian_apply_backward(int P, const float* scaling, const float* rotation, const float* opacity,
                                const float* g_means3D, const float* g_scales, const float* g_rotations,
                                const float* g_opacities, float* d_xyz, float* d_scaling, float* d_rotation,
                                float* d_opacity, float* d_delta, int ld, void* stream);

int dgm_se3_exp_forward(int N, const float* wv, int ld, float* T, void* stream);
int dgm_se3_exp_backward(int N, const float* wv, int ld, const float* dT, float* d_wv, int ldd, void* stream);
int dgm_se3_transform_forward(int N, const float* T, const float* xyz, float* out, void* stream);
int dgm_se3_transform_backward(int N, const float* T, const float* xyz, const float* g_out, float* dT, float* d_xyz, void* stream);

size_t dgm_cycle_loss_workspace_bytes(int N);
int dgm_cycle_loss_forward(int N, const float* a, const float* b, int ld, char* workspace, float* out, void* stream);
int dgm_cycle_loss_backward(int N, const float* a, const float* b, int ld, const float* grad_out, float* d_a, float* d_b,
                            void* stream);


int dgm_adam_step(int n_tensors, float* const* params, const float* const* grads, float* const* exp_avg,
                  float* const* exp_avg_sq, const long long* numel, const float* lr, const int* step, float beta1,
                  float beta2, float eps, void* stream);

int dgm_densify_stats(int P, const float* grad2d, const int* radii, float* max_radii2D, float* grad_accum, float* denom,
                      void* stream);
size_t dgm_densify_scratch_bytes(int P);
size_t dgm_densify_totals_offset(int P);
int dgm_densify_decide(int P, const float* grad_accum, const float* denom, const float* scaling, const float* opacity,
                       float grad_threshold, float dense_extent, float min_opacity, float big_extent,
                       const uint8_t* keep_mask, char* scratch, void* stream);
// ... 106 lines not shown
```

Before: 318.0 it/s.

## Batch deform and deform_back MLP backward into grouped kernels with fused forward addend

Adds a paired forward/backward path for the deform and deform_back networks. The second network's forward adds the first's output to its input inside the embed kernel, and the two backward passes are merged into grouped kernel launches (dout, head gemm, dw, pair, reduce, fold-grad) that process both networks per launch along a grid dimension. The goal is to halve the number of MLP backward launches and fill more of the GPU with the two small, independent workloads. It adds a larger reduce batch struct and a new autograd function, and it is enabled by default through DGM_MLP_GROUP.

```diff
diff --git a/dg-mesh_amd/_lib.py b/dg-mesh_amd/_lib.py
--- a/dg-mesh_amd/_lib.py
+++ b/dg-mesh_amd/_lib.py
@@ -23,6 +23,11 @@
 class MlpParams(_c.Structure):
     _fields_ = [(n, _c.c_int) for n in ("n_layers", "width", "emb_dim", "t_dim", "skip_layer", "n_out")] + [
         ("W", _vp * 8), ("b", _vp * 8), ("Wh", _vp), ("bh", _vp)]
+
+
+class MlpBackwardJob(_c.Structure):
+    _fields_ = [("params", _c.POINTER(MlpParams)), ("dOut", _vp), ("workspace", _vp), ("dW", _vp * 8), ("db", _vp * 8),
+                ("dWh", _vp), ("dbh", _vp), ("dtemb", _vp)]
 
 
 _f, _i = _c.c_float, _c.c_int
@@ -132,8 +137,10 @@
     "dgm_mlp_workspace_bytes": (_c.c_size_t, [_i]),
     "dgm_mlp_describe_workspace": (_i, [_i, _c.POINTER(_c.c_size_t), _i]),
     "dgm_mlp_forward": (_i, [_c.POINTER(MlpParams), _i, _vp, _vp, _i, _vp, _vp, _vp]),
+    "dgm_mlp_forward_add": (_i, [_c.POINTER(MlpParams), _i, _vp, _vp, _i, _vp, _i, _vp, _vp, _vp]),
     "dgm_mlp_backward": (_i, [_c.POINTER(MlpParams), _i, _vp, _i, _vp, _vp * 8, _vp * 8, _vp, _vp, _vp, _vp]),
     "dgm_mlp_backward_dx": (_i, [_c.POINTER(MlpParams), _i, _vp, _i, _vp, _vp * 8, _vp * 8, _vp, _vp, _vp, _vp, _vp, _vp]),
+    "dgm_mlp_backward_group": (_i, [_c.POINTER(MlpBackwardJob), _c.POINTER(MlpBackwardJob), _i, _i, _vp]),
 }
 
 _LIB = None
diff --git a/dg-mesh_amd/csrc/c_api.hip b/dg-mesh_amd/csrc/c_api.hip
--- a/dg-mesh_amd/csrc/c_api.hip
+++ b/dg-mesh_amd/csrc/c_api.hip
@@ -73,6 +73,7 @@
 };
 constexpr int kMaxDeferred = 4096;
 EventPair g_deferred[DGM_STAGE_COUNT][kMaxDeferred];
+int g_deferred_w[DGM_STAGE_COUNT][kMaxDeferred];
 int g_deferred_n[DGM_STAGE_COUNT] = {0};
 int g_deferred_created[DGM_STAGE_COUNT] = {0};
 int g_sample_every = 1;
@@ -118,6 +119,7 @@
                 (void)hipEventCreate(&g_deferred[s][i].b);
                 g_deferred_created[s] = i + 1;
             }
+            g_deferred_w[s][i] = 1;
             (void)hipEventRecord(g_deferred[s][i].a, st);
             used[s] = true;
         }
@@ -146,13 +148,16 @@
 }
 
 namespace dgm {
-void prof_begin(int s, hipStream_t st) {
+void prof_begin(int s, hipStream_t st, int passes) {
     if (g_profile != 2) return;
     std::lock_guard<std::mutex> lk(g_prof_mu);
     g_open[s] = false;
-    if ((g_calls[s]++ % g_sample_every) != 0 || g_deferred_n[s] >= kMaxDeferred) return;
+    const bool sampled = (g_calls[s] % g_sample_every) < passes;
+    g_calls[s] += passes;
+    if (!sampled || g_deferred_n[s] >= kMaxDeferred) return;
     g_open[s] = true;
     const int i = g_deferred_n[s];
+    g_deferred_w[s][i] = passes;
     if (i >= g_deferred_created[s]) {
         (void)hipEventCreate(&g_deferred[s][i].a);
         (void)hipEventCreate(&g_deferred[s][i].b);
@@ -214,7 +219,7 @@
             float ms = 0;
             if (hipEventElapsedTime(&ms, g_deferred[s][i].a, g_deferred[s][i].b) == hipSuccess) {
                 tot += ms;
-                ok++;
+                ok += g_deferred_w[s][i];
             }
         }
         avg_ms[s] = ok ? (float)(tot / ok) : 0.f;
diff --git a/dg-mesh_amd/csrc/mlp.hip b/dg-mesh_amd/csrc/mlp.hip
--- a/dg-mesh_amd/csrc/mlp.hip
+++ b/dg-mesh_amd/csrc/mlp.hip
@@ -283,12 +283,14 @@
 };
 struct ReduceDwBatch {
     int emb_dim, n_jobs;
-    ReduceDwJob job[9];
-    int h_chunks, h_bchunks, h_nout;
-    const float* h_partial_W;
-    const float* h_partial_b;
-    float* h_dW;
-    float* h_db;
+    ReduceDwJob job[18];
+    struct Heads {
+        int chunks, bchunks, nout;
+        const float* partial_W;
+        const float* partial_b;
+        float* dW;
+        float* db;
+    } heads[2];
 };
 __device__ __forceinline__ void reduce_heads_body(int bx, int o, int chunks, int bchunks, const float* __restrict__ partial_W,
                                                   const float* __restrict__ partial_b, float* __restrict__ dWh,
@@ -303,9 +305,10 @@
     constexpr int KT = RDW_KT, JT = RDW_JT, JQ = JT / 4, JB = MLP_W / JT;
     __shared__ float4 red[4][64];
     __shared__ float redb[32][8];
-    if ((int)blockIdx.y == rb.n_jobs) {
-        if ((int)blockIdx.x < 8 * rb.h_nout)
-            reduce_heads_body(blockIdx.x & 7, blockIdx.x >> 3, rb.h_chunks, rb.h_bchunks, rb.h_partial_W, rb.h_partial_b, rb.h_dW, rb.h_db);
+    if ((int)blockIdx.y >= rb.n_jobs) {
+        const ReduceDwBatch::Heads& h = rb.heads[(int)blockIdx.y - rb.n_jobs];
+        if ((int)blockIdx.x < 8 * h.nout)
+            reduce_heads_body(blockIdx.x & 7, blockIdx.x >> 3, h.chunks, h.bchunks, h.partial_W, h.partial_b, h.dW, h.db);
         return;
     }
     const ReduceDwJob& jb = rb.job[blockIdx.y];
@@ -619,7 +622,7 @@
 
 namespace dgm {
 void set_last_error(const char* msg);
-void prof_begin(int stage, hipStream_t st);
+void prof_begin(int stage, hipStream_t st, int passes = 1);
 void prof_end(int stage, hipStream_t st);
 }
 namespace {
@@ -841,7 +844,7 @@
 }
 
 int forward_planes(const dgm_mlp_params* p, int N, const float* x, const float* temb, int temb_stride, const Ws& w, float* out,
-                   hipStream_t st, const bool fold, const bool all5) {
+                   hipStream_t st, const bool fold, const bool all5, const float* xadd = nullptr, const int xadd_stride = 0) {
     const P4Plan pl = p4_plan(N);
     const int nt = pl.ntiles, gx = nt < num_cus() ? nt : num_cus();
     const int sk = p->skip_layer;
@@ -854,7 +857,7 @@
     am.job[8].W = p->Wh, am.job[8].n = p->n_out * MLP_W;
     if (!fold)
         hipLaunchKernelGGL(mlp_embed4_kernel, dim3(nt + 8 * am.n_jobs), dim3(256), 0, st, N, nt, x, temb, temb_stride, p->t_dim,
-                           (unsigned char*)w.emb, w.Eexp, am, w.matmax, EW);
+                           (unsigned char*)w.emb, w.Eexp, am, w.matmax, EW, xadd, xadd_stride);
     if (fold) {
         Prep4cBatch pc;
         int nc = 0;
@@ -877,10 +880,10 @@
         static const bool merged = [] { const char* e = getenv("DGM_MLP_EMBED_MERGED"); return !(e && atoi(e) == 0); }();
         if (merged) {
             const int n_prep = (MLP_W / P4C_COLS) * nc;
-            hipLaunchKernelGGL(mlp_embed4c_kernel, dim3(n_prep + nt), dim3(256), 0, st, N, x, (unsigned char*)w.emb, w.Eexp, EW, pc, n_prep);
+            hipLaunchKernelGGL(mlp_embed4c_kernel, dim3(n_prep + nt), dim3(256), 0, st, N, x, (unsigned char*)w.emb, w.Eexp, EW, pc, n_prep, xadd, xadd_stride);
         } else {
             hipLaunchKernelGGL(mlp_embed4_kernel, dim3(nt), dim3(256), 0, st, N, nt, x, temb, temb_stride, p->t_dim,
-                               (unsigned char*)w.emb, w.Eexp, am, w.matmax, EW);
+                               (unsigned char*)w.emb, w.Eexp, am, w.matmax, EW, xadd, xadd_stride);
             hipLaunchKernelGGL(mlp_prep4c_kernel, dim3(MLP_W / P4C_COLS, nc), dim3(256), 0, st, pc);
         }
     }
@@ -1093,8 +1096,8 @@
         }
     }
     rb.n_jobs = n_pending;
-    rb.h_chunks = pl.chunks, rb.h_bchunks = nt, rb.h_nout = p->n_out, rb.h_partial_W = w.partial_h, rb.h_partial_b = w.partial_hb;
-    rb.h_dW = dWh, rb.h_db = dbh;
+    rb.heads[0].chunks = pl.chunks, rb.heads[0].bchunks = nt, rb.heads[0].nout = p->n_out;
+    rb.heads[0].partial_W = w.partial_h, rb.heads[0].partial_b = w.partial_hb, rb.heads[0].dW = dWh, rb.heads[0].db = dbh;
     hipLaunchKernelGGL(mlp_reduce_dw_all_kernel, dim3(rb_blocks, rb.n_jobs + 1), dim3(256), 0, st, rb);
     if (fold) {
         FoldGradArgs f;
@@ -1105,6 +1108,166 @@
     } else if (dtemb != nullptr && !per_row_t)
         hipLaunchKernelGGL(mlp_dtemb_bcast_kernel, dim3(p->t_dim), dim3(256), 0, st, p->t_dim, db[0], p->W[0], layer_in(p, 0),
                            db[sk], p->W[sk], layer_in(p, sk), dtemb);
+    hipError_t e = hipGetLastError();
+    if (e != hipSuccess) return mlp_fail(hipGetErrorString(e));
+    return 0;
+}
+
+struct GroupNet {
+    const dgm_mlp_params* p;
+    const float* dOut;
+    Ws w;
+    float* const* dW;
+    float* const* db;
+    float *dWh, *dbh, *dtemb;
+};
+int p4_pair_chunks(int N) {
+    const P4Plan pl = p4_plan(N);
+    const int nt = pl.ntiles, gx = nt < num_cus() ? nt : num_cus();
+    int n_dw = p4_pair_split(nt, gx);
+    if (n_dw > pl.chunks) n_dw = pl.chunks;
+    return n_dw;
+}
+int p4_group_split(int N) {
+    const P4Plan pl = p4_plan(N);
+    const int nt = pl.ntiles, gx = nt < num_cus() ? nt : num_cus();
+    const int n_wg = (p4_pair_chunks(N) / 2) & ~7;
+    if (n_wg < 8 || 4 * n_wg > gx) return 0;
+    return n_wg;
+}
+int backward_planes_group(const GroupNet* nets, int N, const int n_wg, hipStream_t st) {
+    const P4Plan pl = p4_plan(N);
+    const int nt = pl.ntiles, sk = 5, EW = 64;
+    const int n_dw = p4_pair_chunks(N);
+    const int cpw = (n_dw + n_wg - 1) / n_wg;
+    const int tpc_s = pl.tiles_per_chunk, chunks_s = pl.chunks;
+    const int tpc_pair = (nt + n_dw - 1) / n_dw, chunks_pair = (nt + tpc_pair - 1) / tpc_pair;
+    {
+        Dout4GroupArgs da;
+        for (int i = 0; i < 2; i++)
+            da.NC[i] = nets[i].p->n_out, da.dOut[i] = nets[i].dOut, da.Dp[i] = nets[i].w.Dp, da.Dexp[i] = nets[i].w.Dexp, da.partial_b[i] = nets[i].w.partial_hb;
+        hipLaunchKernelGGL(mlp_dout4_group_kernel, dim3((nt + 3) / 4, 2), dim3(256), 0, st, N, nt, da);
+    }
+    unsigned char *G[2], *Gn[2];
+    int *Ge[2], *Gne[2];
+    PairGroupArgs pg;
+    memset(&pg, 0, sizeof(pg));
+    for (int i = 0; i < 2; i++) {
+        const Ws& w = nets[i].w;
+        G[i] = (unsigned char*)w.Ga, Gn[i] = (unsigned char*)w.Gb, Ge[i] = w.Gexp[0], Gne[i] = w.Gexp[1];
+        pg.ga[i].ntiles = nt, pg.ga[i].M = N, pg.ga[i].exps_limit = p4_exps_limit();
+        pg.da[i].ntiles = nt;
+    }
+    {
+        Gemm4GroupArgs g7a;
+        for (int i = 0; i < 2; i++) {
+            const Ws& w = nets[i].w;
+            Gemm4Args& a = g7a.a[i];
+            a = pg.ga[i];
+            a.A = w.Dp, a.Aexp = w.Dexp, a.Bp = w.Wh4b, a.b_inv = w.wsc_hb, a.mask_in = w.mask[7], a.C = G[i], a.Cexp = Ge[i];
+        }
+        const int g7 = nt < num_cus() ? nt : num_cus();
+        static bool done_[DGM_MAX_DEVICES] = {false};
+        if (p4_lds_attr(mlp_gemm4_group_kernel<1, 128, 64, 1, false, 8, true>, CfgG7C::LDS, &done_[current_device_slot()]) != hipSuccess)
+            return mlp_fail("mlp: cannot raise the LDS limit of a plane-path kernel");
+        hipLaunchKernelGGL((mlp_gemm4_group_kernel<1, 128, 64, 1, false, 8, true>), dim3(g7, 2), dim3(512), CfgG7C::LDS, st, g7a);
+    }
+    Dw4GroupArgs dg;
+    memset(&dg, 0, sizeof(dg));
+    {
+        for (int i = 0; i < 2; i++) {
+            const Ws& w = nets[i].w;
+            Dw4Args& d = dg.a[i];
+            d.ntiles = nt, d.tiles_per_chunk = tpc_s;
+            d.X = (const unsigned char*)w.Y[7], d.Xexp = w.Yexp[7], d.G = w.Dp, d.Gexp = w.Dexp, d.partial = w.partial_h, d.chunk_stride = 0;
+            d.partial_db = nullptr;
+        }
+        static bool done_[DGM_MAX_DEVICES] = {false};
+        if (p4_lds_attr(mlp_dw4_group_kernel<8, 1, 1024, 512, 128, 64>, CfgDwH::LDS, &done_[current_device_slot()]) != hipSuccess)
+            return mlp_fail("mlp: cannot raise the LDS limit of a plane-path kernel");
+        hipLaunchKernelGGL((mlp_dw4_group_kernel<8, 1, 1024, 512, 128, 64>), dim3(chunks_s, 2), dim3(512), CfgDwH::LDS, st, dg);
+    }
+    ReduceDwBatch rb;
+    memset(&rb, 0, sizeof(rb));
+    rb.emb_dim = nets[0].p->emb_dim;
+    int rb_blocks = 0, n_pending = 0;
+    auto add_job = [&](const dgm_mlp_params* p, int chunks, int db_rows, int Kp, int in_features, int dst_off, const float* partial,
+                       const float* partial_db, float* dWp, float* dbp) {
+        ReduceDwJob& jb = rb.job[n_pending++];
+        jb.chunks = chunks, jb.db_rows = db_rows, jb.Kp = Kp, jb.in_features = in_features, jb.nblocks = reduce_dw_blocks(Kp);
+        jb.emb_rows = EW, jb.k_valid = MLP_XE;
+        jb.dst_off = dst_off, jb.partial = partial, jb.partial_db = partial_db, jb.dW = dWp, jb.db = dbp;
+        if (jb.nblocks > rb_blocks) rb_blocks = jb.nblocks;
+    };
+    for (int l = 7; l >= 0; l--) {
+        if (l == 0 || l == sk) {
+            for (int i = 0; i < 2; i++) {
+                const Ws& w = nets[i].w;
+                Dw4Args& d = dg.a[i];
+                d.ntiles = nt, d.tiles_per_chunk = tpc_s;
+                d.X = (const unsigned char*)w.emb, d.Xexp = w.Eexp, d.G = G[i], d.Gexp = Ge[i];
+                d.partial = l == sk ? w.partial_l[l] + (size_t)n_dw * MLP_W * MLP_W : w.partial_l[l];
+                d.chunk_stride = (size_t)EW * MLP_W, d.partial_db = w.partial_db_l[l];
+                add_job(nets[i].p, chunks_s, 8 * chunks_s, EW, layer_in(nets[i].p, l), 0, d.partial, d.partial_db, nets[i].dW[l], nets[i].db[l]);
+            }
+            static bool done_[DGM_MAX_DEVICES] = {false};
+            if (p4_lds_attr(mlp_dw4_group_kernel<2, 8, 256, 128, 1024, 512>, CfgDwE64::LDS, &done_[current_device_slot()]) != hipSuccess)
+                return mlp_fail("mlp: cannot raise the LDS limit of a plane-path kernel");
+            hipLaunchKernelGGL((mlp_dw4_group_kernel<2, 8, 256, 128, 1024, 512>), dim3(chunks_s, 2), dim3(512), CfgDwE64::LDS, st, dg);
+        }
+        if (l == 0) break;
+        for (int i = 0; i < 2; i++) {
+            const Ws& w = nets[i].w;
+            Gemm4Args& a = pg.ga[i];
+            a.A = G[i], a.Aexp = Ge[i], a.Bp = w.Wd3[l], a.b_inv = w.wsc_d[l], a.mask_in = w.mask[l - 1], a.C = Gn[i], a.Cexp = Gne[i];
+            Dw4Args& d = pg.da[i];
+            d.tiles_per_chunk = tpc_pair;
+            d.X = (const unsigned char*)w.Y[l - 1], d.Xexp = w.Yexp[l - 1], d.G = G[i], d.Gexp = Ge[i];
+            d.partial = w.partial_l[l], d.chunk_stride = (size_t)MLP_W * MLP_W;
+            d.partial_db = l == sk ? nullptr : w.partial_db_l[l];
+            if (l == sk)
+                add_job(nets[i].p, chunks_pair, 0, MLP_W, layer_in(nets[i].p, l), nets[i].p->emb_dim, d.partial, nullptr, nets[i].dW[l], nullptr);
+            else
+                add_job(nets[i].p, chunks_pair, 8 * chunks_pair, MLP_W, layer_in(nets[i].p, l), 0, d.partial, d.partial_db, nets[i].dW[l], nets[i].db[l]);
+        }
+        dgm::prof_begin(DGM_STAGE_MLP_BWD_PAIR, st, 2);
+        {
+            static bool done_[DGM_MAX_DEVICES] = {false};
+            constexpr int LDS_PAIR = CfgBwdC::LDS > CfgDw::LDS ? CfgBwdC::LDS : CfgDw::LDS;
+            if (p4_lds_attr(mlp_bwd_pair_group_kernel<true>, LDS_PAIR, &done_[current_device_slot()]) != hipSuccess)
+                return mlp_fail("mlp: cannot raise the LDS limit of mlp_bwd_pair_group_kernel");
+            hipLaunchKernelGGL(mlp_bwd_pair_group_kernel<true>, dim3(4 * n_wg), dim3(512), LDS_PAIR, st, pg, n_wg, cpw, n_dw);
+        }
+        dgm::prof_end(DGM_STAGE_MLP_BWD_PAIR, st);
+        for (int i = 0; i < 2; i++) {
+            unsigned char* t = G[i];
+            G[i] = Gn[i], Gn[i] = t;
+            int* te = Ge[i];
+            Ge[i] = Gne[i], Gne[i] = te;
+        }
+    }
+    rb.n_jobs = n_pending;
+    for (int i = 0; i < 2; i++) {
+        ReduceDwBatch::Heads& h = rb.heads[i];
+        h.chunks = chunks_s, h.bchunks = nt, h.nout = nets[i].p->n_out;
+        h.partial_W = nets[i].w.partial_h, h.partial_b = nets[i].w.partial_hb, h.dW = nets[i].dWh, h.db = nets[i].dbh;
+    }
+    hipLaunchKernelGGL(mlp_reduce_dw_all_kernel, dim3(rb_blocks, rb.n_jobs + 2), dim3(256), 0, st, rb);
+    {
+        FoldGradGroupArgs fg;
+        int tmax = 0;
+        bool any_dt = false;
+        for (int i = 0; i < 2; i++) {
+            const dgm_mlp_params* p = nets[i].p;
+            FoldGradArgs& f = fg.f[i];
+            f.dW[0] = nets[i].dW[0], f.db[0] = nets[i].db[0], f.W[0] = p->W[0], f.in_features[0] = layer_in(p, 0);
+            f.dW[1] = nets[i].dW[sk], f.db[1] = nets[i].db[sk], f.W[1] = p->W[sk], f.in_features[1] = layer_in(p, sk);
+            f.temb = nets[i].w.temb_row, f.T = p->t_dim, f.dtemb = nets[i].dtemb;
+            if (p->t_dim > tmax) tmax = p->t_dim;
+            any_dt = any_dt || f.dtemb != nullptr;
+        }
+        hipLaunchKernelGGL(mlp_fold_grad_group_kernel, dim3(any_dt ? 3 : 2, tmax, 2), dim3(256), 0, st, fg);
+    }
     hipError_t e = hipGetLastError();
     if (e != hipSuccess) return mlp_fail(hipGetErrorString(e));
     return 0;
@@ -1250,15 +1413,22 @@
 
 int dgm_mlp_forward(const dgm_mlp_params* p, int N, const float* x, const float* temb, int temb_stride, char* workspace,
                     float* out, void* stream) {
+    return dgm_mlp_forward_add(p, N, x, nullptr, 0, temb, temb_stride, workspace, out, stream);
+}
+
+int dgm_mlp_forward_add(const dgm_mlp_params* p, int N, const float* x, const float* x_add, int x_add_stride, const float* temb,
+                        int temb_stride, char* workspace, float* out, void* stream) {
     if (check_params(p)) return 1;
     if (N <= 0) return 0;
     if (!x || !temb || !workspace || !out) return mlp_fail("mlp_forward: NULL pointer");
+    if (x_add && (g_gemm_mode < 3 || x_add_stride < 3))
+        return mlp_fail("mlp_forward_add: the addend exists in the plane arithmetic only (f16x3p), rows of at least 3 floats");
     hipStream_t st = (hipStream_t)stream;
     Ws w = carve(workspace, N);
     const int mode = g_gemm_mode;
     const bool fold = (mode == 3 || mode == 5) && temb_stride == 0;
     remember_ws_mode(workspace, mode + (fold ? 16 : 0));
-    if (mode >= 3) return forward_planes(p, N, x, temb, temb_stride, w, out, st, fold, fold && mode == 5);
+    if (mode >= 3) return forward_planes(p, N, x, temb, temb_stride, w, out, st, fold, fold && mode == 5, x_add, x_add_stride);
     for (int l = 0; l < 8; l++) {
         const int Kp = layer_kp(p, l);
         const int n = (Kp > MLP_W ? Kp : MLP_W) * MLP_W;
@@ -1362,6 +1532,35 @@
     return 0;
 }
 
+int dgm_mlp_backward_group(const dgm_mlp_backward_job* a, const dgm_mlp_backward_job* b, int N, int temb_stride, void* stream) {
+    if (!a || !b) return mlp_fail("mlp_backward_group: NULL job");
+    const dgm_mlp_backward_job* jobs[2] = {a, b};
+    if (check_params(a->params) || check_params(b->params)) return 1;
+    if (N <= 0) return 0;
+    for (const dgm_mlp_backward_job* j : jobs)
+        if (!j->dOut || !j->workspace || !j->dWh || !j->dbh) return mlp_fail("mlp_backward_group: NULL pointer");
+    if (a->workspace == b->workspace) return mlp_fail("mlp_backward_group: the two networks need workspaces of their own");
+    const int mode = g_gemm_mode;
+    const int fa = recall_ws_mode(a->workspace), fb = recall_ws_mode(b->workspace);
+    const int n_wg = p4_group_split(N);
+    const bool grouped = n_wg > 0 && mode == 3 && temb_stride == 0 && fa == (3 | 16) && fb == (3 | 16) &&
+                         a->params->emb_dim == b->params->emb_dim;
+    if (!grouped) {
+        for (const dgm_mlp_backward_job* j : jobs)
+            if (dgm_mlp_backward(j->params, N, j->dOut, temb_stride, j->workspace, j->dW, j->db, j->dWh, j->dbh, j->dtemb, stream)) return 1;
+        return 0;
+    }
+    GroupNet nets[2];
+    for (int i = 0; i < 2; i++) {
+        const dgm_mlp_backward_job* j = jobs[i];
+        for (int l = 0; l < 8; l++)
+            if (!j->dW[l] || !j->db[l]) return mlp_fail("mlp_backward_group: NULL gradient pointer");
+        nets[i].p = j->params, nets[i].dOut = j->dOut, nets[i].w = carve(j->workspace, N);
+        nets[i].dW = j->dW, nets[i].db = j->db, nets[i].dWh = j->dWh, nets[i].dbh = j->dbh, nets[i].dtemb = j->dtemb;
+    }
+    return backward_planes_group(nets, N, n_wg, (hipStream_t)stream);
+}
+
 int dgm_timenet_forward(const float* t, int n_freq, const float* W1, const float* b1, int hidden, const float* W2,
                         const float* b2, int n_out, float* save, float* out, void* stream) {
     if (!t || !W1 || !b1 || !W2 || !b2 || !save || !out) return mlp_fail("timenet_forward: NULL pointer");
diff --git a/dg-mesh_amd/csrc/mlp_planes.hpp b/dg-mesh_amd/csrc/mlp_planes.hpp
--- a/dg-mesh_amd/csrc/mlp_planes.hpp
+++ b/dg-mesh_amd/csrc/mlp_planes.hpp
@@ -140,11 +140,12 @@
 
 __device__ __forceinline__ void embed4_tile(const int N, const int tile, const float* __restrict__ x, const float* __restrict__ temb,
                                             const int temb_stride, const int T, unsigned char* __restrict__ Ep, int* __restrict__ Eexp,
-                                            const int EW, float (*se)[96 + 1], float* smax);
+                                            const int EW, float (*se)[96 + 1], float* smax, const float* __restrict__ xadd = nullptr,
+                                            const int xadd_stride = 0);
 __global__ void __launch_bounds__(256)
 mlp_embed4_kernel(int N, int ntiles, const float* __restrict__ x, const float* __restrict__ temb, int temb_stride, int T,
                   unsigned char* __restrict__ Ep, int* __restrict__ Eexp, const AbsMaxBatch am, unsigned* __restrict__ matmax,
-                  const int EW) {
+                  const int EW, const float* __restrict__ xadd, const int xadd_stride) {
     __shared__ float se[32][96 + 1];
     __shared__ float smax[4];
     const int tid = threadIdx.x, lane = tid & 63, wv = tid >> 6;
@@ -174,11 +175,12 @@
         if (tid == 0) matmax[job * AS + part] = __float_as_uint(fmaxf(fmaxf(smax[0], smax[1]), fmaxf(smax[2], smax[3])));
         return;
     }
-    embed4_tile(N, (int)blockIdx.x - n_am, x, temb, temb_stride, T, Ep, Eexp, EW, se, smax);
+    embed4_tile(N, (int)blockIdx.x - n_am, x, temb, temb_stride, T, Ep, Eexp, EW, se, smax, xadd, xadd_stride);
 }
 __device__ __forceinline__ void embed4_tile(const int N, const int tile, const float* __restrict__ x, const float* __restrict__ temb,
                                             const int temb_stride, const int T, unsigned char* __restrict__ Ep, int* __restrict__ Eexp,
-                                            const int EW, float (*se)[96 + 1], float* smax) {
+                                            const int EW, float (*se)[96 + 1], float* smax, const float* __restrict__ xadd,
+                                            const int xadd_stride) {
     const int tid = threadIdx.x, lane = tid & 63, wv = tid >> 6;
     const int r0 = tile * 32;
     float mx = 0.f;
@@ -188,7 +190,11 @@
             const int sub = lane / 30, p = lane - 30 * sub, rl = 8 * wv + 2 * it + sub, r = r0 + rl;
             const int q = p / 3, a = p - 3 * q;
             float sn = 0.f, cs = 0.f;
-            if (r < N) sincosf(x[3 * r + a] * (float)(1 << q), &sn, &cs);
+            if (r < N) {
+                float xv = x[3 * r + a];
+                if (xadd != nullptr) xv += xadd[(size_t)r * xadd_stride + a];
+                sincosf(xv * (float)(1 << q), &sn, &cs);
+            }
             se[rl][3 + 6 * q + a] = sn;
             se[rl][6 + 6 * q + a] = cs;
         }
@@ -200,7 +206,10 @@
         int c;
         if (j < 3) {
             c = j;
-            if (r < N) v = x[3 * r + j];
+            if (r < N) {
+                v = x[3 * r + j];
+                if (xadd != nullptr) v += xadd[(size_t)r * xadd_stride + j];
+            }
         } else {
             const int t = j - 3;
             c = 63 + t;
@@ -345,19 +354,18 @@
 }
 __global__ void __launch_bounds__(256)
 mlp_embed4c_kernel(const int N, const float* __restrict__ x, unsigned char* __restrict__ Ep, int* __restrict__ Eexp, const int EW,
-                   const Prep4cBatch b, const int n_prep) {
+                   const Prep4cBatch b, const int n_prep, const float* __restrict__ xadd, const int xadd_stride) {
     if ((int)blockIdx.x < n_prep) {
         prep4c_block(b, (int)blockIdx.x % (256 / P4C_COLS), (int)blockIdx.x / (256 / P4C_COLS));
         return;
     }
     __shared__ float se[32][96 + 1];
     __shared__ float smax[4];
-    embed4_tile(N, (int)blockIdx.x - n_prep, x, nullptr, 0, 0, Ep, Eexp, EW, se, smax);
-}
-
-__global__ void __launch_bounds__(256)
-mlp_dout4_kernel(int N, int ntiles, int NC, const float* __restrict__ dOut, unsigned char* __restrict__ Dp, int* __restrict__ Dexp,
-                 float* __restrict__ partial_b) {
+    embed4_tile(N, (int)blockIdx.x - n_prep, x, nullptr, 0, 0, Ep, Eexp, EW, se, smax, xadd, xadd_stride);
+}
+
+__device__ __forceinline__ void dout4_body(int N, int ntiles, int NC, const float* __restrict__ dOut, unsigned char* __restrict__ Dp,
+                                           int* __restrict__ Dexp, float* __restrict__ partial_b) {
     const int lane = threadIdx.x & 63, wv = threadIdx.x >> 6;
     const int tile = blockIdx.x * 4 + wv;
     if (tile >= ntiles) return;
@@ -393,6 +401,11 @@
         for (int dd = 16; dd >= 1; dd >>= 1) s += __shfl_xor(s, dd, 64);
         if (rl == 0) partial_b[(size_t)tile * 16 + 8 * hf + i] = s;
     }
+}
+__global__ void __launch_bounds__(256)
+mlp_dout4_kernel(int N, int ntiles, int NC, const float* __restrict__ dOut, unsigned char* __restrict__ Dp, int* __restrict__ Dexp,
+                 float* __restrict__ partial_b) {
+    dout4_body(N, ntiles, NC, dOut, Dp, Dexp, partial_b);
 }
 
 struct Gemm4Args {
@@ -921,7 +934,9 @@
     if (nst <= 0) return;
 
     int eref = 0x7fffffff;
-    for (int t = t0; t < t1; t++) eref = min(eref, a.Xexp[t] + a.Gexp[t]);
+    for (int t = t0 + lane; t < t1; t += 64) eref = min(eref, a.Xexp[t] + a.Gexp[t]);
+#pragma unroll
+    for (int d = 32; d >= 1; d >>= 1) eref = min(eref, __shfl_xor(eref, d, 64));
     eref = __builtin_amdgcn_readfirstlane(eref);
 
     const bool isX = tid < XB, isG = tid >= 256 && tid < 256 + GB;
@@ -1112,6 +1127,65 @@
     }
 }
 
+struct PairGroupArgs {
+    Gemm4Args ga[2];
+    Dw4Args da[2];
+};
+template <bool COLSC>
+__global__ void __launch_bounds__(512)
+mlp_bwd_pair_group_kernel(const PairGroupArgs s, const int n_wg, const int cpw, const int n_chunks) {
+    extern __shared__ __attribute__((aligned(16))) unsigned char p4_smem[];
+    const int net = __builtin_amdgcn_readfirstlane((int)blockIdx.x >= 2 * n_wg ? 1 : 0);
+    const int w = (int)blockIdx.x - net * 2 * n_wg;
+    if (w < n_wg) {
+        const Dw4Args& da = s.da[net];
+        const int c1 = min(n_chunks, (w + 1) * cpw);
+#pragma unroll 1
+        for (int c = w * cpw; c < c1; c++) {
+            dw4_body<8, 8, 1024, 512, 1024, 512>(da, c, p4_smem);
+            __syncthreads();
+        }
+    } else {
+        const Gemm4Args& ga = s.ga[net];
+        const int span = s.da[net].tiles_per_chunk * cpw;
+        const int first = (w - n_wg) * span;
+        const int cnt = min(span, ga.ntiles - first);
+        gemm4_body<16, 1024, 512, 1, false, 8, COLSC>(ga, first, 1, p4_smem, cnt > 0 ? cnt : 0);
+    }
+}
+struct Dw4GroupArgs {
+    Dw4Args a[2];
+};
+template <int MT, int NT, int XROWB, int XPLANEB, int GROWB, int GPLANEB>
+__global__ void __launch_bounds__(512)
+mlp_dw4_group_kernel(const Dw4GroupArgs s) {
+    extern __shared__ __attribute__((aligned(16))) unsigned char p4_smem[];
+    const Dw4Args a = s.a[__builtin_amdgcn_readfirstlane((int)blockIdx.y)];
+    dw4_body<MT, NT, XROWB, XPLANEB, GROWB, GPLANEB>(a, (int)blockIdx.x, p4_smem);
+}
+struct Gemm4GroupArgs {
+    Gemm4Args a[2];
+};
+template <int KS, int ROWB, int PLANEB, int EPI, bool DUAL, int NCW, bool COLSC = false>
+__global__ void __launch_bounds__(512)
+mlp_gemm4_group_kernel(const Gemm4GroupArgs s) {
+    extern __shared__ __attribute__((aligned(16))) unsigned char p4_smem[];
+    const Gemm4Args a = s.a[__builtin_amdgcn_readfirstlane((int)blockIdx.y)];
+    gemm4_body<KS, ROWB, PLANEB, EPI, DUAL, NCW, COLSC>(a, (int)blockIdx.x, (int)gridDim.x, p4_smem);
+}
+struct Dout4GroupArgs {
+    int NC[2];
+    const float* dOut[2];
+    unsigned char* Dp[2];
+    int* Dexp[2];
+    float* partial_b[2];
+};
+__global__ void __launch_bounds__(256)
+mlp_dout4_group_kernel(int N, int ntiles, const Dout4GroupArgs s) {
+    const int i = blockIdx.y;
+    dout4_body(N, ntiles, s.NC[i], s.dOut[i], s.Dp[i], s.Dexp[i], s.partial_b[i]);
+}
+
 __global__ void __launch_bounds__(256)
 mlp_dx4_kernel(int N, const unsigned char* __restrict__ G, const int* __restrict__ Gexp, const float* __restrict__ W, int in_features,
                int col0, int ncol, float* __restrict__ scratch, int finish, const float* __restrict__ x, float* __restrict__ dX,
diff --git a/dg-mesh_amd/csrc/mlp_planes5.hpp b/dg-mesh_amd/csrc/mlp_planes5.hpp
--- a/dg-mesh_amd/csrc/mlp_planes5.hpp
+++ b/dg-mesh_amd/csrc/mlp_planes5.hpp
@@ -441,8 +441,21 @@
     float* dtemb;
     int T;
 };
+__device__ __forceinline__ void fold_grad_body(const FoldGradArgs& f);
 __global__ void __launch_bounds__(256)
 mlp_fold_grad_kernel(const FoldGradArgs f) {
+    fold_grad_body(f);
+}
+struct FoldGradGroupArgs {
+    FoldGradArgs f[2];
+};
+__global__ void __launch_bounds__(256)
+mlp_fold_grad_group_kernel(const FoldGradGroupArgs s) {
+    const FoldGradArgs& f = s.f[blockIdx.z];
+    if ((int)blockIdx.y >= f.T || (blockIdx.x == 2 && f.dtemb == nullptr)) return;
+    fold_grad_body(f);
+}
+__device__ __forceinline__ void fold_grad_body(const FoldGradArgs& f) {
     __shared__ float red[4];
     const int k = blockIdx.x, t = blockIdx.y, j = threadIdx.x;
     if (k < 2) {
diff --git a/dg-mesh_amd/deform.py b/dg-mesh_amd/deform.py
--- a/dg-mesh_amd/deform.py
+++ b/dg-mesh_amd/deform.py
@@ -253,6 +253,24 @@
         self.net.load_state_dict(torch.load(os.path.join(root, f"iteration_{iteration}/{self.model_name}.pth")))
 
 
+def step_raw_pair(model, model_back, xyz, time_emb, time_emb_back):
+    net, net_back = model.net, model_back.net
+    for n in (net, net_back):
+        if not isinstance(n, DeformNetwork) or n.is_6dof or n.trunk_impl != "hip":
+            return None
+    if not xyz.is_cuda or xyz.requires_grad:
+        return None
+    for t in (time_emb, time_emb_back):
+        if not (t.dim() == 2 and t.shape[0] > 1 and t.stride(0) == 0):
+            return None
+    from . import mlp_hip
+    if not mlp_hip.pair_supported(xyz, True, True):
+        return None
+    t_a, _ = net._time_rows(time_emb)
+    t_b, _ = net_back._time_rows(time_emb_back)
+    return mlp_hip.network_pair_forward(net, net.head_modules(), net_back, net_back.head_modules(), xyz, t_a, t_b)
+
+
 class DeformModel(_ModelWrapper):
     def __init__(self, is_blender=False, is_6dof=False, device="cuda", trunk_impl=None):
         super().__init__(DeformNetwork(is_blender=is_blender, is_6dof=is_6dof, trunk_impl=trunk_impl).to(device), 5, "deform")
diff --git a/dg-mesh_amd/mlp_hip.py b/dg-mesh_amd/mlp_hip.py
--- a/dg-mesh_amd/mlp_hip.py
+++ b/dg-mesh_amd/mlp_hip.py
@@ -102,6 +102,74 @@
                                               ctypes.c_void_p(dbh.data_ptr()), ctypes.c_void_p(dtemb.data_ptr()), st))
         dWs, dbs = torch.split(dWh, head_rows, 0), torch.split(dbh, head_rows, 0)
         return (dX, dtemb if need_t else None, None, None, *dWs, *dbs, *dW, *db)
+
+
+def _unpack(tensors, n_heads):
+    hw, hb, wb = tensors[:n_heads], tensors[n_heads:2 * n_heads], tensors[2 * n_heads:]
+    n_out = sum(w.shape[0] for w in hw)
+    Wh, bh = _stacked(hw, (n_out, hw[0].shape[1])), _stacked(hb, (n_out,))
+    return Wh, bh, [w.contiguous() for w in wb[:8]], [v.contiguous() for v in wb[8:]], [w.shape[0] for w in hw]
+
+
+class _MLPPairFunction(torch.autograd.Function):
+
+    @staticmethod
+    def forward(ctx, x, t_a, t_b, nh_a, nh_b, *tensors):
+        L = _lib.lib()
+        n_a = 2 * nh_a + 16
+        nets = [_unpack(tensors[:n_a], nh_a), _unpack(tensors[n_a:], nh_b)]
+        x = x.contiguous()
+        N = x.shape[0]
+        vp = lambda t: ctypes.c_void_p(t.data_ptr())
+        st = _lib.stream_ptr()
+        outs, wss, saved = [], [], []
+        with _lib.device_guard(x.device):
+            for i, ((Wh, bh, W, b, _), t) in enumerate(zip(nets, (t_a.contiguous(), t_b.contiguous()))):
+                ws = torch.empty(L.dgm_mlp_workspace_bytes(N), dtype=torch.uint8, device=x.device)
+                out = torch.empty((N, Wh.shape[0]), dtype=torch.float32, device=x.device)
+                p = _params(None, W, b, Wh, bh, t.shape[1])
+                if i == 0:
+                    _lib.check(L.dgm_mlp_forward(ctypes.byref(p), N, vp(x), vp(t), 0, vp(ws), vp(out), st))
+                else:
+                    _lib.check(L.dgm_mlp_forward_add(ctypes.byref(p), N, vp(x), vp(outs[0]), outs[0].shape[1], vp(t), 0, vp(ws),
+                                                     vp(out), st))
+                outs.append(out)
+                wss.append(ws)
+                saved += [ws, Wh, bh, *W, *b]
+        ctx.save_for_backward(*saved)
+        ctx.meta = (N, (t_a.shape[1], t_b.shape[1]), (t_a.requires_grad, t_b.requires_grad), (nets[0][4], nets[1][4]))
+        return outs[0], outs[1]
+
+    @staticmethod
+    def backward(ctx, dOut_a, dOut_b):
+        L = _lib.lib()
+        N, Ts, need_t, head_rows = ctx.meta
+        saved = ctx.saved_tensors
+        dev = saved[0].device
+        jobs, keep, grads, dtembs = [], [], [], []
+        for i, dOut in enumerate((dOut_a, dOut_b)):
+            ws, Wh, bh, *wb = saved[19 * i:19 * (i + 1)]
+            W, b = wb[:8], wb[8:]
+            if dOut is None:
+                dOut = torch.zeros((N, Wh.shape[0]), dtype=torch.float32, device=dev)
+            dOut = dOut.contiguous()
+            dW = [torch.empty_like(w) for w in W]
+            db = [torch.empty_like(v) for v in b]
+            dWh, dbh = torch.empty_like(Wh), torch.empty_like(bh)
+            dtemb = torch.empty((1, Ts[i]), dtype=torch.float32, device=dev)
+            p = _params(None, W, b, Wh, bh, Ts[i])
+            j = _lib.MlpBackwardJob()
+            j.params, j.dOut, j.workspace = ctypes.pointer(p), dOut.data_ptr(), ws.data_ptr()
+            for l in range(8):
+                j.dW[l], j.db[l] = dW[l].data_ptr(), db[l].data_ptr()
+            j.dWh, j.dbh, j.dtemb = dWh.data_ptr(), dbh.data_ptr(), dtemb.data_ptr()
+            jobs.append(j)
+            keep.append((p, dOut))
+            dtembs.append(dtemb if need_t[i] else None)
+            grads += [*torch.split(dWh, head_rows[i], 0), *torch.split(dbh, head_rows[i], 0), *dW, *db]
+        with _lib.device_guard(dev):
+            _lib.check(L.dgm_mlp_backward_group(ctypes.byref(jobs[0]), ctypes.byref(jobs[1]), N, 0, _lib.stream_ptr()))
+        return (None, dtembs[0], dtembs[1], None, None, *grads)
 
 
 class _TimeNetFunction(torch.autograd.Function):
@@ -179,3 +247,16 @@
     W = [l.weight for l in net.linear]
     b = [l.bias for l in net.linear]
     return _MLPFunction.apply(x, t_emb, bcast, len(heads), *[m.weight for m in heads], *[m.bias for m in heads], *W, *b)
+
+
+def pair_supported(x, bcast_a, bcast_b):
+    return (x.is_cuda and not x.requires_grad and bcast_a and bcast_b and _lib.lib().dgm_mlp_set_gemm(-1) in (3, 4, 5))
+
+
+def network_pair_forward(net_a, heads_a, net_b, heads_b, x, t_emb_a, t_emb_b):
+    check_supported(net_a, heads_a, t_emb_a)
+    check_supported(net_b, heads_b, t_emb_b)
+    flat = []
+    for net, heads in ((net_a, heads_a), (net_b, heads_b)):
+        flat += [m.weight for m in heads] + [m.bias for m in heads] + [l.weight for l in net.linear] + [l.bias for l in net.linear]
+    return _MLPPairFunction.apply(x, t_emb_a, t_emb_b, len(heads_a), len(heads_b), *flat)
diff --git a/dg-mesh_amd/trainer.py b/dg-mesh_amd/trainer.py
--- a/dg-mesh_amd/trainer.py
+++ b/dg-mesh_amd/trainer.py
@@ -155,8 +155,10 @@
     def __init__(self, gaussians, deform, deform_back, cameras, opt=None, pipe=None, background=None,
                  is_blender=True, is_6dof=False, rank=0, world=1, seed=0, render_fn=None, fused_adam=None,
                  process_group=None, fused_loss=True, fused_glue=None, track_stats=True, densify=False,
-                 cameras_extent=1.0, prune_threshold=0.005, white_background=True, overlap=False, mesh=None):
+                 cameras_extent=1.0, prune_threshold=0.005, white_background=True, overlap=False, mesh=None,
+                 group_mlp_backward=None):
         self.g, self.deform, self.deform_back = gaussians, deform, deform_back
+        self.group_mlp_backward = (os.environ.get("DGM_MLP_GROUP", "1") != "0") if group_mlp_backward is None else bool(group_mlp_backward)
         self.mesh = mesh
         self.cameras = cameras
         self.opt = opt or S.OptimizationParams()
@@ -368,7 +370,13 @@
             N = g.get_xyz.shape[0]
             time_input = self.time_input(cam, N, iteration)
             t_back = self.time_input(cam, N, iteration)
-            if self.fused_glue:
+            back = None
+            if self.fused_glue and self.group_mlp_backward:
+                from .deform import step_raw_pair
+                pair = step_raw_pair(self.deform, self.deform_back, g.get_xyz.detach(), time_input, t_back)
+                if pair is not None:
+                    delta, back = pair
+            if self.fused_glue and delta is None:
                 delta = self.deform.step_raw(g.get_xyz.detach(), time_input)
             if delta is None:
                 d_xyz, d_rotation, d_scaling = self.deform.step(g.get_xyz.detach(), time_input)[:3]
@@ -376,7 +384,10 @@
         if delta is not None:
             from .glue import cycle_loss
             lean = {"lean": True} if self.render_fn is S.render else {}
-            if self.world > 1 and self._early is not None:
+            if back is not None:
+                pkg = self.render_fn(cam, g, self.pipe, self.bg, None, None, None, self.is_6dof, delta=delta, **lean)
+                losses["cycle_loss"] = cycle_loss(delta, back)
+            elif self.world > 1 and self._early is not None:
                 means = (g.get_xyz.detach() + delta.detach()[:, :3]).contiguous()
                 back = self.deform_back.step_raw(means, t_back)
                 losses["cycle_loss"] = cycle_loss(delta, back)
diff --git a/include/dgmesh_hip.h b/include/dgmesh_hip.h
--- a/include/dgmesh_hip.h
+++ b/include/dgmesh_hip.h
@@ -150,11 +150,26 @@
 int dgm_mlp_forward(const dgm_mlp_params* p, int N, const float* x, const float* temb, int temb_stride,
                     char* workspace, float* out, void* stream);
 
+int dgm_mlp_forward_add(const dgm_mlp_params* p, int N, const float* x, const float* x_add, int x_add_stride, const float* temb,
+                        int temb_stride, char* workspace, float* out, void* stream);
+
 int dgm_mlp_backward(const dgm_mlp_params* p, int N, const float* dOut, int temb_stride, char* workspace,
                      float* const* dW, float* const* db, float* dWh, float* dbh, float* dtemb, void* stream);
 int dgm_mlp_backward_dx(const dgm_mlp_params* p, int N, const float* dOut, int temb_stride, char* workspace,
                         float* const* dW, float* const* db, float* dWh, float* dbh, float* dtemb, const float* x, float* dX,
                         void* stream);
+
+typedef struct {
+    const dgm_mlp_params* params;
+    const float* dOut;
+    char* workspace;
+    float* dW[8];
+    float* db[8];
+    float* dWh;
+    float* dbh;
+    float* dtemb;
+} dgm_mlp_backward_job;
+int dgm_mlp_backward_group(const dgm_mlp_backward_job* a, const dgm_mlp_backward_job* b, int N, int temb_stride, void* stream);
 
 int dgm_timenet_forward(const float* t, int n_freq, const float* W1, const float* b1, int hidden, const float* W2,
                         const float* b2, int n_out, float* save, float* out, void* stream);
```

After: 326.4 it/s, median of 6. 1.03x the previous value.
